# stefan01/Fusion-Method-for-Video-Frame-Interpolation

Measured on AMD Instinct MI355X. Metric: interpolated frames/sec at 1080p, higher is better.
Workload: dtype f32; 1 GPU; full fused frame (PhaseNet + 4x AdaCoF + uncertainty maps + FusionNet, output_baseline) at 1920x1080, BASELINE.json configs[3]; one frame pair per rank per step; weights=random-init, 22940546 params broadcast from rank 0, frames_in_flight_per_gpu=3, hip_graph=False

## Files before the change

### fusion-method-for-video-frame-interpolation_amd/csrc/vfi_adacof.hip

```cpp
#include "vfi_grad_common.h"

#include <cstdlib>

namespace {

using vfi::ceil_div;

template <int VEC>
struct Vec;
template <>
struct Vec<1> {
    float v[1];
    __device__ __forceinline__ void load(const float *p) { v[0] = *p; }
};
template <>
struct Vec<4> {
    float v[4];
    __device__ __forceinline__ void load(const float *p) {
        const float4 t = *reinterpret_cast<const float4 *>(p);
        v[0] = t.x; v[1] = t.y; v[2] = t.z; v[3] = t.w;
    }
};

template <>
// ... 100 lines not shown
    float acc[VEC][C];
#pragma unroll
    for (int v = 0; v < VEC; ++v)
#pragma unroll
        for (int c = 0; c < C; ++c) acc[v][c] = 0.0f;

    for (int k = 0; k < F; ++k)
        for (int l = 0; l < F; ++l) {
            const size_t t = tbase + (size_t)(k * F + l) * plane;
            Vec<VEC> w, a, b;
            w.load(weight + t);
            a.load(offset_i + t);
            b.load(offset_j + t);
#pragma unroll
            for (int v = 0; v < VEC; ++v)
                tap_accumulate<C>(in, in_plane, Hin, Win, y + k * dil, x0 + v + l * dil, w.v[v],
                                  a.v[v], b.v[v], acc[v]);
        }
#pragma unroll
    for (int c = 0; c < C; ++c) {
        if (c0 + c < Ctot) {
            float o[VEC];
#pragma unroll
            for (int v = 0; v < VEC; ++v) o[v] = acc[v][c];
            store_vec<VEC>(output + ((size_t)n * Ctot + c0 + c) * plane + pix, o);
        }
    }
}

struct FlowStats {
    float m, q;
};

template <int C, int VEC, int FT, int UNROLL_L, int MIN_WAVES, bool RGBX = false, bool SOFTMAX = false, bool WIN = false>
__global__ __launch_bounds__(256, MIN_WAVES) void adacof_fused_kernel(
    const float *__restrict__ frame0, const float *__restrict__ frame2,
    const float *__restrict__ w1, const float *__restrict__ a1, const float *__restrict__ b1,
    const float *__restrict__ w2, const float *__restrict__ a2, const float *__restrict__ b2,
    const float *__restrict__ occ, float *__restrict__ out_t1, float *__restrict__ out_t2,
    float *__restrict__ out_frame, float *__restrict__ out_mask, int H, int W, int Frt, int dil, int margin) {
    const int F = FT > 0 ? FT : Frt;
    const int x0 = (blockIdx.x * 64 + threadIdx.x) * VEC;
    const int y = blockIdx.y * 4 + threadIdx.y;
    const int n = blockIdx.z;
    extern __shared__ float4 win_lds[];
    const int WH = 4 + (F - 1) * dil + 2 * margin + 1, WW = 64 + (F - 1) * dil + 2 * margin + 1;
    const int yb = blockIdx.y * 4 - ((F - 1) * dil) / 2 - margin, xb = blockIdx.x * 64 - ((F - 1) * dil) / 2 - margin;
    if constexpr (WIN) {
        const int tid = threadIdx.y * 64 + threadIdx.x;
        const float4 *g0 = reinterpret_cast<const float4 *>(frame0) + (size_t)n * H * W;
        const float4 *g2 = reinterpret_cast<const float4 *>(frame2) + (size_t)n * H * W;
        for (int e = tid; e < WH * WW; e += 256) {
            const int gy = min(max(yb + e / WW, 0), H - 1), gx = min(max(xb + e % WW, 0), W - 1);
            win_lds[e] = g0[gy * W + gx];
            win_lds[WH * WW + e] = g2[gy * W + gx];
        }
        __syncthreads();
    }
    if (x0 >= W || y >= H) return;
    const size_t plane = (size_t)H * W;
    const size_t pix = (size_t)y * W + x0;
    const size_t tbase = (size_t)n * F * F * plane + pix;
    const int pad = ((F - 1) * dil) / 2;

    float res[2][VEC][C];
    float var[2][VEC];
    float acc[VEC][C], s[VEC], pa[VEC], pb[VEC], mx[VEC];
    FlowStats sa[VEC], sb[VEC];
    auto side_begin = [&](const Vec<VEC> &a0, const Vec<VEC> &b0) {
#pragma unroll
        for (int v = 0; v < VEC; ++v) {
#pragma unroll
            for (int c = 0; c < C; ++c) acc[v][c] = 0.0f;
// ... 112 lines not shown
#pragma unroll
            for (int l = 0; l < FT; ++l) { cw[l] = nw[l]; ca[l] = na[l]; cb[l] = nb[l]; }
        }
    } else {
#pragma unroll
        for (int side = 0; side < 2; ++side) {
            const float *__restrict__ in = (side ? frame2 : frame0) + (size_t)n * (RGBX ? 4 : C) * plane;
            const float *__restrict__ wp = side ? w2 : w1;
            const float *__restrict__ ap = side ? a2 : a1;
            const float *__restrict__ bp = side ? b2 : b1;
            {
                Vec<VEC> a, b;
                a.load(ap + tbase);
                b.load(bp + tbase);
                side_begin(a, b);
            }
#pragma unroll 1
            for (int k = 0; k < F; ++k)
#pragma unroll UNROLL_L
                for (int l = 0; l < F; ++l) {
                    const size_t t = tbase + (size_t)(k * F + l) * plane;
                    Vec<VEC> w, a, b;
                    w.load(wp + t);
                    a.load(ap + t);
                    b.load(bp + t);
                    tap(side, in, k, l, w, a, b);
                }
            side_end(res[side], var[side]);
        }
    }

    Vec<VEC> o;
    o.load(occ + (size_t)n * plane + pix);
#pragma unroll
    for (int c = 0; c < C; ++c) {
        const size_t q = ((size_t)n * C + c) * plane + pix;
        float f[VEC], t1[VEC], t2[VEC];
#pragma unroll
        for (int v = 0; v < VEC; ++v) {
            t1[v] = res[0][v][c];
            t2[v] = res[1][v][c];
            f[v] = o.v[v] * t1[v] + (1.0f - o.v[v]) * t2[v];
        }
        store_vec<VEC>(out_frame + q, f);
        if (out_t1) store_vec<VEC>(out_t1 + q, t1);
        if (out_t2) store_vec<VEC>(out_t2 + q, t2);
    }
    if (out_mask) {
        float m[VEC];
#pragma unroll
        for (int v = 0; v < VEC; ++v) {
            const float mx = fmaxf(var[0][v], var[1][v]);
            m[v] = fminf(fmaxf(mx, 0.0f), 20.0f) / 20.0f;
        }
        store_vec<VEC>(out_mask + (size_t)n * plane + pix, m);
    }
}

template <int CT>
__device__ __forceinline__ void tap_gradient(const float *__restrict__ in, size_t in_plane, int C, int Hin, int Win,
                                             int row, int col, float alpha, float beta, const float *dreg,
                                             const float *__restrict__ dglob, size_t plane, float &gw, float &sa,
                                             float &sb) {
    const int A = (int)alpha;
    const int B = (int)beta;
    const float fa = alpha - (float)A;
// ... 104 lines not shown
                                   float *grad_offset_i, float *grad_offset_j, int N, int C, int Hin, int Win,
                                   int H, int W, int F, int dilation, vfi_stream_t stream) {
    const bool want_off = grad_offset_i || grad_offset_j;
    VFI_REQUIRE(grad_weight || want_off, VFI_ERR_INVALID_ARG, "vfi_adacof_backward: no gradient requested");
    VFI_REQUIRE(grad_output && input && offset_i && offset_j && (weight || !want_off), VFI_ERR_INVALID_ARG,
                "vfi_adacof_backward: null pointer");
    VFI_REQUIRE(N > 0 && C > 0 && H > 0 && W > 0 && F > 0 && dilation > 0, VFI_ERR_INVALID_ARG,
                "vfi_adacof_backward: non-positive size");
    VFI_REQUIRE(Hin - ((F - 1) * dilation + 1) == H - 1 && Win - ((F - 1) * dilation + 1) == W - 1,
                VFI_ERR_SHAPE, "vfi_adacof_backward: input %dx%d does not match output %dx%d for F=%d dilation=%d",
                Hin, Win, H, W, F, dilation);
    VFI_REQUIRE((long long)Hin * Win < (1ll << 31) && (long long)N * F * F * H * W < (1ll << 40) &&
                    (long long)N * C * Hin * Win < (1ll << 40),
                VFI_ERR_UNSUPPORTED, "vfi_adacof_backward: tensor too large");
    if (!want_off) weight = nullptr;
    hipStream_t s = vfi::as_stream(stream);
    dim3 block(64, 4);
    dim3 grid(vfi::ceil_div(W, 64), vfi::ceil_div(H, 4), N);
    VFI_REQUIRE(grid.z <= 65535 && grid.y <= 65535, VFI_ERR_UNSUPPORTED, "vfi_adacof_backward: grid too large");
#define LAUNCH(CT)                                                                                           \
    hipLaunchKernelGGL((adacof_backward_kernel<CT, 1>), grid, block, 0, s, grad_output, input, weight, offset_i, \
                       offset_j, grad_weight, grad_offset_i, grad_offset_j, C, Hin, Win, H, W, F, dilation)
    if (C == 3) LAUNCH(3);
    else if (C == 1) LAUNCH(1);
    else LAUNCH(0);
#undef LAUNCH
    return vfi::check_launch("vfi_adacof_backward");
}

static int adacof_fused_impl(const float *frame0, const float *frame2, const float *w1,
                             const float *a1, const float *b1, const float *w2, const float *a2,
                             const float *b2, const float *occ, float *out_t1, float *out_t2,
                             float *out_frame, float *out_mask, int N, int C, int H, int W, int F,
                             int dilation, bool rgbx, bool softmax, vfi_stream_t stream) {
    VFI_REQUIRE(frame0 && frame2 && w1 && a1 && b1 && w2 && a2 && b2 && occ && out_frame,
                VFI_ERR_INVALID_ARG, "vfi_adacof_fused: null pointer");
    VFI_REQUIRE(N > 0 && H > 0 && W > 0 && F > 0 && dilation > 0, VFI_ERR_INVALID_ARG,
                "vfi_adacof_fused: non-positive size");
    VFI_REQUIRE(C == 3, VFI_ERR_UNSUPPORTED, "vfi_adacof_fused: C=%d (only 3 colour channels)", C);
    VFI_REQUIRE(((F - 1) * dilation) % 2 == 0, VFI_ERR_SHAPE,
                "vfi_adacof_fused: (F-1)*dilation must be even (F=%d dilation=%d)", F, dilation);
    VFI_REQUIRE((long long)H * W < (1ll << 31), VFI_ERR_UNSUPPORTED, "vfi_adacof_fused: frame too large");
    bool al16 = aligned16(occ) && aligned16(out_frame);
    for (const void *p : {(const void *)w1, (const void *)a1, (const void *)b1, (const void *)w2,
                          (const void *)a2, (const void *)b2})
        al16 = al16 && aligned16(p);
    for (const void *p : {(const void *)out_t1, (const void *)out_t2, (const void *)out_mask})
        al16 = al16 && (p == nullptr || aligned16(p));
    static const int variant = getenv("VFI_ADACOF_VARIANT") ? atoi(getenv("VFI_ADACOF_VARIANT")) : 2;
    int vec = (al16 && W % 4 == 0) ? 4 : ((al16 && W % 2 == 0) ? 2 : 1);
    if (variant == 1 && vec == 4) vec = 2;
    if (variant == 2 || rgbx) vec = 1;
    if (rgbx) VFI_REQUIRE(aligned16(frame0) && aligned16(frame2), VFI_ERR_INVALID_ARG, "vfi_adacof_fused_rgbx: frames must be 16-B aligned");
    hipStream_t s = vfi::as_stream(stream);
    dim3 block(64, 4);
    dim3 grid(vfi::ceil_div(W, 64 * vec), vfi::ceil_div(H, 4), N);
    VFI_REQUIRE(grid.z <= 65535 && grid.y <= 65535, VFI_ERR_UNSUPPORTED, "vfi_adacof_fused: grid too large");
#define LAUNCH(VEC, FT, UN, MW)                                                                          \
    hipLaunchKernelGGL((adacof_fused_kernel<3, VEC, FT, UN, MW>), grid, block, 0, s, frame0, frame2, w1, a1, b1, \
                       w2, a2, b2, occ, out_t1, out_t2, out_frame, out_mask, H, W, F, dilation, 0)
    if (softmax) VFI_REQUIRE(rgbx, VFI_ERR_UNSUPPORTED, "vfi_adacof_fused: softmax folding needs the rgbx entry point");
    static const int win_margin = getenv("VFI_ADACOF_MARGIN") ? atoi(getenv("VFI_ADACOF_MARGIN")) : 4;
    const int wh = 4 + (F - 1) * dilation + 2 * win_margin + 1, ww = 64 + (F - 1) * dilation + 2 * win_margin + 1;
    const size_t win_bytes = 2ull * wh * ww * sizeof(float4);
    if (rgbx && win_margin > 0 && win_bytes <= 64 * 1024) {
#define LAUNCH_WIN(FT, UN, SM)                                                                                       \
    hipLaunchKernelGGL((adacof_fused_kernel<3, 1, FT, UN, 3, true, SM, true>), grid, block, win_bytes, s, frame0, frame2, w1, \
                       a1, b1, w2, a2, b2, occ, out_t1, out_t2, out_frame, out_mask, H, W, F, dilation, win_margin)
        if (F == 5) { if (softmax) LAUNCH_WIN(5, 5, true); else LAUNCH_WIN(5, 5, false); }
        else        { if (softmax) LAUNCH_WIN(0, 1, true); else LAUNCH_WIN(0, 1, false); }
#undef LAUNCH_WIN
    } else if (rgbx) {
        if (F == 5 && softmax)
            hipLaunchKernelGGL((adacof_fused_kernel<3, 1, 5, 5, 3, true, true>), grid, block, 0, s, frame0, frame2, w1, a1, b1,
                               w2, a2, b2, occ, out_t1, out_t2, out_frame, out_mask, H, W, F, dilation, 0);
        else if (softmax)
            hipLaunchKernelGGL((adacof_fused_kernel<3, 1, 0, 1, 4, true, true>), grid, block, 0, s, frame0, frame2, w1, a1, b1,
                               w2, a2, b2, occ, out_t1, out_t2, out_frame, out_mask, H, W, F, dilation, 0);
        else if (F == 5)
            hipLaunchKernelGGL((adacof_fused_kernel<3, 1, 5, 5, 3, true>), grid, block, 0, s, frame0, frame2, w1, a1, b1,
                               w2, a2, b2, occ, out_t1, out_t2, out_frame, out_mask, H, W, F, dilation, 0);
        else
            hipLaunchKernelGGL((adacof_fused_kernel<3, 1, 0, 1, 4, true>), grid, block, 0, s, frame0, frame2, w1, a1, b1,
                               w2, a2, b2, occ, out_t1, out_t2, out_frame, out_mask, H, W, F, dilation, 0);
    } else if (F == 5) {
        if (vec == 4) LAUNCH(4, 5, 1, 3);
        else if (vec == 2) LAUNCH(2, 5, 1, 4);
        else LAUNCH(1, 5, 5, 3);
    } else {
        if (vec == 4) LAUNCH(4, 0, 1, 3); else if (vec == 2) LAUNCH(2, 0, 1, 4); else LAUNCH(1, 0, 1, 4);
    }
#undef LAUNCH
    return vfi::check_launch("vfi_adacof_fused");
}

extern "C" int vfi_adacof_fused(const float *frame0, const float *frame2, const float *w1,
                                const float *a1, const float *b1, const float *w2, const float *a2,
                                const float *b2, const float *occ, float *out_t1, float *out_t2,
                                float *out_frame, float *out_mask, int N, int C, int H, int W, int F,
                                int dilation, vfi_stream_t stream) {
    return adacof_fused_impl(frame0, frame2, w1, a1, b1, w2, a2, b2, occ, out_t1, out_t2, out_frame, out_mask, N, C,
                             H, W, F, dilation, false, false, stream);
}

extern "C" int vfi_adacof_fused_rgbx(const float *frame0_rgbx, const float *frame2_rgbx, const float *w1,
                                     const float *a1, const float *b1, const float *w2, const float *a2,
                                     const float *b2, const float *occ, float *out_t1, float *out_t2,
                                     float *out_frame, float *out_mask, int N, int H, int W, int F,
                                     int dilation, int weights_are_logits, vfi_stream_t stream) {
    return adacof_fused_impl(frame0_rgbx, frame2_rgbx, w1, a1, b1, w2, a2, b2, occ, out_t1, out_t2, out_frame,
                             out_mask, N, 3, H, W, F, dilation, true, weights_are_logits != 0, stream);
}
```

### fusion-method-for-video-frame-interpolation_amd/csrc/vfi_aux.hip

```cpp
#include "vfi_grad_common.h"

namespace {

using vfi::ceil_div;

__global__ void adacof_prepare_kernel(const float *__restrict__ f0, const float *__restrict__ f2,
                                      float *__restrict__ p0, float *__restrict__ p2, float *__restrict__ x6,
                                      int N, int H, int W, int Hp, int Wp, int rgbx) {
    const long long total = (long long)N * 3 * Hp * Wp;
    for (long long i = (long long)blockIdx.x * blockDim.x + threadIdx.x; i < total; i += (long long)gridDim.x * blockDim.x) {
        const int x = i % Wp, y = (i / Wp) % Hp, c = (i / ((long long)Wp * Hp)) % 3, n = i / ((long long)Wp * Hp * 3);
        const int sy = y < H ? y : 2 * (H - 1) - y, sx = x < W ? x : 2 * (W - 1) - x;
        const size_t s = (((size_t)n * 3 + c) * H + sy) * W + sx;
        const float mean = c == 0 ? 0.4631f : (c == 1 ? 0.4352f : 0.3990f);
        const float a = f0[s], b = f2[s];
        const size_t plane = (size_t)Hp * Wp, pix = (size_t)y * Wp + x;
        if (rgbx) {
            p0[((size_t)n * plane + pix) * 4 + c] = a;
            p2[((size_t)n * plane + pix) * 4 + c] = b;
        } else {
            p0[i] = a;
            p2[i] = b;
        }
        x6[((size_t)n * 6 + c) * plane + pix] = a - mean;
        x6[((size_t)n * 6 + 3 + c) * plane + pix] = b - mean;
    }
}

template <bool MAX>
__global__ void pool2_kernel(const float *__restrict__ x, long long x_bs, float *__restrict__ y, long long y_bs,
                             int N, int C, int H, int W) {
    const int Ho = H / 2, Wo = W / 2;
    const long long total = (long long)N * C * Ho * Wo;
    for (long long i = (long long)blockIdx.x * blockDim.x + threadIdx.x; i < total; i += (long long)gridDim.x * blockDim.x) {
        const int xo = i % Wo, yo = (i / Wo) % Ho, c = (i / ((long long)Wo * Ho)) % C, n = i / ((long long)Wo * Ho * C);
        const float *p = x + (size_t)n * x_bs + ((size_t)c * H + 2 * yo) * W + 2 * xo;
        const float2 r0 = *reinterpret_cast<const float2 *>(p);
        const float2 r1 = *reinterpret_cast<const float2 *>(p + W);
        const float v = MAX ? fmaxf(fmaxf(r0.x, r0.y), fmaxf(r1.x, r1.y)) : (r0.x + r0.y + r1.x + r1.y) * 0.25f;
        y[(size_t)n * y_bs + ((size_t)c * Ho + yo) * Wo + xo] = v;
    }
}
template <bool MAX>
__global__ void pool2_kernel_unaligned(const float *__restrict__ x, long long x_bs, float *__restrict__ y,
                                       long long y_bs, int N, int C, int H, int W) {
    const int Ho = H / 2, Wo = W / 2;
    const long long total = (long long)N * C * Ho * Wo;
    for (long long i = (long long)blockIdx.x * blockDim.x + threadIdx.x; i < total; i += (long long)gridDim.x * blockDim.x) {
        const int xo = i % Wo, yo = (i / Wo) % Ho, c = (i / ((long long)Wo * Ho)) % C, n = i / ((long long)Wo * Ho * C);
        const float *p = x + (size_t)n * x_bs + ((size_t)c * H + 2 * yo) * W + 2 * xo;
        const float a = p[0], b = p[1], cc = p[W], d = p[W + 1];
        const float v = MAX ? fmaxf(fmaxf(a, b), fmaxf(cc, d)) : (a + b + cc + d) * 0.25f;
        y[(size_t)n * y_bs + ((size_t)c * Ho + yo) * Wo + xo] = v;
    }
}
// ... 262 lines not shown
}
__global__ void phasenet_emit_low_fuse_kernel(const float *__restrict__ pred, long long pred_bs, const float *__restrict__ low,
                                              long long low_bs, const float *__restrict__ maxv, float *__restrict__ out,
                                              int N, int HW) {
    const long long total = (long long)N * HW;
    for (long long i = (long long)blockIdx.x * blockDim.x + threadIdx.x; i < total; i += (long long)gridDim.x * blockDim.x) {
        const int p = i % HW, n = i / HW;
        const float *pr = pred + (size_t)n * pred_bs + p;
        const float alpha = (pr[0] + 1.0f) / 2.0f, fa = (pr[HW] + 1.0f) / 2.0f;
        const float *l = low + (size_t)n * low_bs + p;
        const float two = alpha * l[0] + (1.0f - alpha) * l[HW];
        out[i] = (fa * two + (1.0f - fa) * l[(size_t)2 * HW]) * maxv[n];
    }
}

__global__ void tanh_residual_clamp_kernel(const float *__restrict__ x, const float *__restrict__ base,
                                           float *__restrict__ y, long long total) {
    for (long long i = (long long)blockIdx.x * blockDim.x + threadIdx.x; i < total; i += (long long)gridDim.x * blockDim.x)
        y[i] = fminf(fmaxf(base[i] + tanhf(x[i]), 0.0f), 1.0f);
}

}

extern "C" int vfi_adacof_prepare(const float *frame0, const float *frame2, float *pad0, float *pad2, float *x6,
                                  int N, int H, int W, int Hp, int Wp, int rgbx, vfi_stream_t stream) {
    VFI_REQUIRE(frame0 && frame2 && pad0 && pad2 && x6, VFI_ERR_INVALID_ARG, "vfi_adacof_prepare: null pointer");
    VFI_REQUIRE(N > 0 && H > 0 && W > 0 && Hp >= H && Wp >= W, VFI_ERR_INVALID_ARG, "vfi_adacof_prepare: bad sizes");
    VFI_REQUIRE(Hp - H < H && Wp - W < W, VFI_ERR_SHAPE, "vfi_adacof_prepare: reflect pad %dx%d needs a larger frame than %dx%d",
                Hp - H, Wp - W, H, W);
    LAUNCH_1D(adacof_prepare_kernel, (long long)N * 3 * Hp * Wp, stream, frame0, frame2, pad0, pad2, x6, N, H, W, Hp, Wp, rgbx);
    return vfi::check_launch("vfi_adacof_prepare");
}

extern "C" int vfi_pool2(const float *x, long long x_bstride, float *y, long long y_bstride, int N, int C, int H,
                         int W, int is_max, vfi_stream_t stream) {
    VFI_REQUIRE(x && y, VFI_ERR_INVALID_ARG, "vfi_pool2: null pointer");
    VFI_REQUIRE(N > 0 && C > 0 && H >= 2 && W >= 2, VFI_ERR_INVALID_ARG, "vfi_pool2: bad sizes");
    const long long total = (long long)N * C * (H / 2) * (W / 2);
    const bool al = (W % 2 == 0) && ((reinterpret_cast<uintptr_t>(x) & 7u) == 0) && (x_bstride % 2 == 0);
    if (al) {
        if (is_max) LAUNCH_1D(pool2_kernel<true>, total, stream, x, x_bstride, y, y_bstride, N, C, H, W);
        else LAUNCH_1D(pool2_kernel<false>, total, stream, x, x_bstride, y, y_bstride, N, C, H, W);
    } else {
        if (is_max) LAUNCH_1D(pool2_kernel_unaligned<true>, total, stream, x, x_bstride, y, y_bstride, N, C, H, W);
        else LAUNCH_1D(pool2_kernel_unaligned<false>, total, stream, x, x_bstride, y, y_bstride, N, C, H, W);
    }
    return vfi::check_launch("vfi_pool2");
}

extern "C" int vfi_resize_bilinear(const float *x, long long x_bstride, const float *residual, long long res_bstride,
                                   float *y, long long y_bstride, int N, int C, int Hin, int Win, int Hout, int Wout,
                                   int align_corners, int relu_input, vfi_stream_t stream) {
    VFI_REQUIRE(x && y, VFI_ERR_INVALID_ARG, "vfi_resize_bilinear: null pointer");
    VFI_REQUIRE(N > 0 && C > 0 && Hin > 0 && Win > 0 && Hout > 0 && Wout > 0, VFI_ERR_INVALID_ARG,
                "vfi_resize_bilinear: bad sizes");
    const bool vec = Wout % 4 == 0 && (reinterpret_cast<uintptr_t>(y) & 15u) == 0 && y_bstride % 4 == 0 &&
                     (!residual || ((reinterpret_cast<uintptr_t>(residual) & 15u) == 0 && res_bstride % 4 == 0));
    VFI_REQUIRE((long long)N * C <= 65535, VFI_ERR_UNSUPPORTED, "vfi_resize_bilinear: N*C = %lld planes", (long long)N * C);
    const dim3 block(64, 4), grid(ceil_div(vec ? Wout / 4 : Wout, 64), ceil_div(Hout, 4), N * C);
    if (Hin <= Hout && Win <= Wout && Hout >= kRsTileY && Wout >= 64) {
        const dim3 tgrid(ceil_div(Wout, kRsTileX), ceil_div(Hout, kRsTileY), N * C);
        if (vec)
            hipLaunchKernelGGL(resize_bilinear_tile_kernel<true>, tgrid, dim3(256), 0, vfi::as_stream(stream), x, x_bstride, residual,
                               res_bstride, y, y_bstride, C, Hin, Win, Hout, Wout, align_corners, relu_input);
        else
            hipLaunchKernelGGL(resize_bilinear_tile_kernel<false>, tgrid, dim3(256), 0, vfi::as_stream(stream), x, x_bstride, residual,
// ... 108 lines not shown
```

### fusion-method-for-video-frame-interpolation_amd/csrc/vfi_conv.hip

```cpp
#include "vfi_conv_common.h"

#include <cstdlib>

using namespace vfi::conv;

namespace {

using f32x16 = __attribute__((ext_vector_type(16))) float;


__device__ float g_zero_word = 0.0f;



template <int KS, int CK, int NT, int RW = 2>
struct ConvTile {
    static constexpr int TH = 4 * RW, TW = 32, PADK = (KS - 1) / 2;
    static constexpr int R = TH + KS - 1, PW = TW + KS - 1, PLANE = R * PW, TAPS = KS * KS, BN = 32 * NT;
    static constexpr int IN_ELEMS = CK * PLANE;
    static constexpr int IN_ELEMS_PAD = (IN_ELEMS + 3) / 4 * 4;
    static constexpr int W_ELEMS = CK * TAPS * BN;
    static constexpr int IN_PER_THREAD = (IN_ELEMS + 255) / 256;
    static constexpr int W4_PER_THREAD = (W_ELEMS / 4 + 255) / 256;
    static constexpr int W_ALLOC = (W_ELEMS + 255) / 256 * 256;
// ... 350 lines not shown
    vec *yp = reinterpret_cast<vec *>(y + (size_t)blockIdx.y * y_bs) + q;
#pragma unroll
    for (int o = 0; o < NOUT; ++o) {
        if (o < Cout) {
            const float b = bias ? bias[o] : 0.0f;
            vec r;
#pragma unroll
            for (int k = 0; k < VEC; ++k) r[k] = apply_act(acc[o][k] + b, a_);
            yp[(size_t)o * plane] = r;
        }
    }
}

static int conv1x1_stream_vec(const ConvArgs &a, int KS) {
    static const bool on = !(getenv("VFI_CONV_STREAM1X1") && atoi(getenv("VFI_CONV_STREAM1X1")) == 0);
    const long long HW = (long long)a.H * a.W;
    if (!on || KS != 1 || a.Cout > 16 || a.res || HW < 4096) return 0;
    const uintptr_t bits = reinterpret_cast<uintptr_t>(a.x) | reinterpret_cast<uintptr_t>(a.y) | (uintptr_t)(a.x_bs * 4) | (uintptr_t)(a.y_bs * 4) |
                           (uintptr_t)(HW * 4);
    return (bits & 15u) == 0 ? 4 : (bits & 7u) == 0 ? 2 : 0;
}

template <int NOUT, int VEC>
static int launch_conv1x1_stream(const ConvArgs &a, int N, hipStream_t s) {
    const int HW = a.H * a.W;
    const dim3 grid((unsigned)vfi::ceil_div(HW / VEC, 256), (unsigned)N);
    if (a.act == 3)
        hipLaunchKernelGGL((conv1x1_stream_kernel<3, NOUT, VEC>), grid, dim3(256), 0, s, a.x, a.x_bs, a.wp, a.bias, a.y, a.y_bs, a.Cin, a.Cout, a.Cout_pad, HW, a.act);
    else
        hipLaunchKernelGGL((conv1x1_stream_kernel<-1, NOUT, VEC>), grid, dim3(256), 0, s, a.x, a.x_bs, a.wp, a.bias, a.y, a.y_bs, a.Cin, a.Cout, a.Cout_pad, HW, a.act);
    return vfi::check_launch("vfi_conv2d");
}

template <int VEC>
__global__ __launch_bounds__(256) void phasenet_predict_kernel(const float *__restrict__ x, long long x_bs, const float *__restrict__ wp,
                                                               const float *__restrict__ bias, int Cout_pad, const float *__restrict__ amp_in,
                                                               long long amp_bs, const float *__restrict__ maxv, float *__restrict__ pred,
                                                               long long pred_bs, float *__restrict__ phase_out, float *__restrict__ amp_out,
                                                               int Cin, int HW) {
    typedef float vec __attribute__((ext_vector_type(VEC)));
    const int q = blockIdx.x * 256 + threadIdx.x;
    if (q * VEC >= HW) return;
    const int n = blockIdx.y;
    const vec *xp = reinterpret_cast<const vec *>(x + (size_t)n * x_bs) + q;
    const size_t plane = (size_t)HW / VEC;
    float acc[8][VEC];
#pragma unroll
    for (int o = 0; o < 8; ++o)
#pragma unroll
        for (int k = 0; k < VEC; ++k) acc[o][k] = 0.0f;
    int c = 0;
    for (; c + 8 <= Cin; c += 8) {
        vec v[8];
#pragma unroll
        for (int i = 0; i < 8; ++i) v[i] = xp[(size_t)(c + i) * plane];
#pragma unroll
        for (int i = 0; i < 8; ++i) {
            const float *w = wp + (size_t)(c + i) * Cout_pad;
#pragma unroll
            for (int o = 0; o < 8; ++o) {
                const float wo = w[o];
#pragma unroll
                for (int k = 0; k < VEC; ++k) acc[o][k] = fmaf(wo, v[i][k], acc[o][k]);
            }
        }
    }
    for (; c < Cin; ++c) {
        const vec v = xp[(size_t)c * plane];
        const float *w = wp + (size_t)c * Cout_pad;
#pragma unroll
        for (int o = 0; o < 8; ++o) {
            const float wo = w[o];
#pragma unroll
            for (int k = 0; k < VEC; ++k) acc[o][k] = fmaf(wo, v[k], acc[o][k]);
        }
    }
    vec *pp = reinterpret_cast<vec *>(pred + (size_t)n * pred_bs) + q;
#pragma unroll
    for (int o = 0; o < 8; ++o) {
        const float b = bias ? bias[o] : 0.0f;
        vec r;
#pragma unroll
        for (int k = 0; k < VEC; ++k) r[k] = acc[o][k] = apply_act(acc[o][k] + b, 3);
        pp[(size_t)o * plane] = r;
    }
    const vec *ap = reinterpret_cast<const vec *>(amp_in + (size_t)n * amp_bs) + q;
    vec *pho = reinterpret_cast<vec *>(phase_out + (size_t)n * 4 * HW) + q, *amo = reinterpret_cast<vec *>(amp_out + (size_t)n * 4 * HW) + q;
    const float mx = maxv[n];
#pragma unroll
    for (int b = 0; b < 4; ++b) {
        const vec a0 = ap[(size_t)b * plane], a1 = ap[(size_t)(4 + b) * plane];
        vec ph, am;
#pragma unroll
        for (int k = 0; k < VEC; ++k) {
            const float beta = (acc[4 + b][k] + 1.0f) / 2.0f;
            const float a = fmaf(beta, a1[k], (1.0f - beta) * a0[k]);
            ph[k] = acc[b][k] * 3.14159265358979323846f;
            am[k] = a * mx;
        }
        pho[(size_t)b * plane] = ph;
        amo[(size_t)b * plane] = am;
    }
}

template <int VEC>
__global__ __launch_bounds__(256) void phasenet_predict_fuse_kernel(const float *__restrict__ x, long long x_bs, const float *__restrict__ wp,
                                                                    const float *__restrict__ bias, int Cout_pad, const float *__restrict__ amp_in,
                                                                    long long amp_bs, const float *__restrict__ maxv, float *__restrict__ pred,
                                                                    long long pred_bs, float *__restrict__ phase_out, float *__restrict__ amp_out,
                                                                    int Cin, int HW) {
    typedef float vec __attribute__((ext_vector_type(VEC)));
    constexpr int NOUT = 12;
    const int q = blockIdx.x * 256 + threadIdx.x;
    if (q * VEC >= HW) return;
    const int n = blockIdx.y;
    const vec *xp = reinterpret_cast<const vec *>(x + (size_t)n * x_bs) + q;
    const size_t plane = (size_t)HW / VEC;
// ... 70 lines not shown
        hipLaunchKernelGGL(conv2d_splitk_reduce_kernel<1>, dim3(vfi::ceil_div(HW, 256), b.Cout, N), dim3(256), 0, s, b.ws,
                           b.splits, b.bias, b.res, b.res_bs, b.y, b.y_bs, b.Cout, HW, b.act);
}

extern "C" long long vfi_conv2d_packed_floats(int Cout, int Cin, int KS) {
    if (Cout <= 0 || Cin <= 0 || KS <= 0) return -1;
    return (long long)round_up(Cin, 8) * (KS * KS + (KS == 3 ? 16 + 36 : 0)) * round_up(Cout, 32);
}

extern "C" int vfi_conv2d_pack(const float *w_oihw, const float *scale, float *packed, int Cout, int Cin,
                               int KS, vfi_stream_t stream) {
    VFI_REQUIRE(w_oihw && packed, VFI_ERR_INVALID_ARG, "vfi_conv2d_pack: null pointer");
    VFI_REQUIRE(Cout > 0 && Cin > 0 && (KS == 1 || KS == 3 || KS == 5), VFI_ERR_INVALID_ARG,
                "vfi_conv2d_pack: bad shape Cout=%d Cin=%d KS=%d", Cout, Cin, KS);
    const int Cin_pad = round_up(Cin, 8), Cout_pad = round_up(Cout, 32);
    const long long total = (long long)Cin_pad * KS * KS * Cout_pad;
    const int blocks = (int)((total + 255) / 256 < 4096 ? (total + 255) / 256 : 4096);
    hipLaunchKernelGGL(conv2d_pack_kernel, dim3(blocks), dim3(256), 0, vfi::as_stream(stream), w_oihw, scale,
                       packed, Cout, Cin, KS * KS, Cin_pad, Cout_pad);
    if (KS == 3) {
        launch_pack_winograd(w_oihw, scale, packed + total, Cout, Cin, Cin_pad, Cout_pad, vfi::as_stream(stream));
        launch_pack_winograd4(w_oihw, scale, packed + total + (long long)Cin_pad * 16 * Cout_pad, Cout, Cin, Cin_pad, Cout_pad,
                              vfi::as_stream(stream));
    }
    return vfi::check_launch("vfi_conv2d_pack");
}

static int conv2d_impl(const float *x, long long x_bstride, const float *packed_w, const float *bias,
                       const float *residual, long long res_bstride, float *y, long long y_bstride, int N,
                       int Cin, int H, int W, int Cout, int KS, int pad_mode, int act, bool ups, float *workspace,
                       long long workspace_floats, vfi_stream_t stream, const float *x2 = nullptr, long long x2_bstride = 0,
                       int rsz_channels = 0, int Hs = 0, int Ws = 0, float *pooled = nullptr, long long pooled_bstride = 0,
                       int pool_max = 0) {
    VFI_REQUIRE(x && packed_w && y, VFI_ERR_INVALID_ARG, "vfi_conv2d: null pointer");
    VFI_REQUIRE(N > 0 && Cin > 0 && Cout > 0 && H > 0 && W > 0, VFI_ERR_INVALID_ARG, "vfi_conv2d: non-positive size");
    VFI_REQUIRE(KS == 1 || KS == 3 || KS == 5, VFI_ERR_UNSUPPORTED, "vfi_conv2d: kernel size %d", KS);
    VFI_REQUIRE(pad_mode == 0 || pad_mode == 1, VFI_ERR_INVALID_ARG, "vfi_conv2d: pad_mode %d", pad_mode);
    VFI_REQUIRE(act >= 0 && act <= 4, VFI_ERR_INVALID_ARG, "vfi_conv2d: act %d", act);
    VFI_REQUIRE(pad_mode == 0 || ((KS - 1) / 2 < H && (KS - 1) / 2 < W), VFI_ERR_SHAPE,
                "vfi_conv2d: reflect padding %d needs a larger input than %dx%d", (KS - 1) / 2, H, W);
    VFI_REQUIRE((long long)Cin * H * W < (1ll << 31) && (long long)Cout * H * W < (1ll << 31), VFI_ERR_UNSUPPORTED,
                "vfi_conv2d: per-sample tensor too large for 32-bit offsets");
    VFI_REQUIRE(N <= 65535, VFI_ERR_UNSUPPORTED, "vfi_conv2d: batch %d", N);
    ConvArgs a;
    a.x = x; a.wp = packed_w; a.bias = bias; a.res = residual; a.y = y;
    a.x_bs = x_bstride; a.res_bs = res_bstride; a.y_bs = y_bstride;
    a.Cin = Cin; a.Cin_pad = round_up(Cin, 8); a.Cout = Cout; a.Cout_pad = round_up(Cout, 32);
    a.H = H; a.W = W; a.tiles_x = vfi::ceil_div(W, 32);
    a.pad_mode = pad_mode; a.act = act;
    a.ws = workspace_floats > 0 ? workspace : nullptr; a.ws_floats = workspace ? workspace_floats : 0; a.splits = 1;
    a.x2 = nullptr; a.x2_bs = 0; a.rsz_channels = 0; a.wino_tiles = 0; a.wino_items = 0; a.wino_batch = 0; a.wino_run = 1;
    a.Hs = H / 2; a.Ws = W / 2;
    a.pool = nullptr; a.pool_bs = 0; a.pool_max = pool_max;
    a.ups_sy = H > 1 ? (float)(a.Hs - 1) / (float)(H - 1) : 0.0f;
    a.ups_sx = W > 1 ? (float)(a.Ws - 1) / (float)(W - 1) : 0.0f;
    hipStream_t s = vfi::as_stream(stream);
    const bool wide = (a.Cout_pad % 64 == 0);
    if (ups) {
        VFI_REQUIRE(KS == 3 && pad_mode == 0 && H % 2 == 0 && W % 2 == 0 && H < 65536 && W < 65536, VFI_ERR_UNSUPPORTED,
                    "vfi_conv2d_upsample2x: needs KS=3, zero padding, even output size (got KS=%d pad=%d %dx%d)", KS, pad_mode, H, W);
        return wide ? launch_conv<3, 8, 2, 1>(a, N, s) : launch_conv<3, 8, 1, 1>(a, N, s);
    }
    if (x2) {
        VFI_REQUIRE(KS == 3 && wide && rsz_channels > 0 && rsz_channels % 8 == 0 && rsz_channels <= Cin && Hs > 0 && Ws > 0 &&
                    H < 65536 && W < 65536, VFI_ERR_UNSUPPORTED,
                    "vfi_conv2d_resized_prefix: needs KS=3, Cout%%64==0, prefix channels a multiple of 8 (got KS=%d Cout=%d prefix=%d)",
                    KS, Cout, rsz_channels);
        a.x2 = x2; a.x2_bs = x2_bstride; a.rsz_channels = rsz_channels; a.Hs = Hs; a.Ws = Ws;
        a.ups_sy = (float)Hs / (float)H; a.ups_sx = (float)Ws / (float)W;
        return launch_conv<3, 8, 2, 2>(a, N, s);
    }
    static const bool wino_on = !(getenv("VFI_CONV_WINOGRAD") && atoi(getenv("VFI_CONV_WINOGRAD")) == 0);
    const long long wino_work_items = (long long)a.tiles_x * vfi::ceil_div(H, 8) * N * (a.Cout_pad / 32) * 16;
    if (KS == 3 && wino_on && (long long)Cin * H * W * 4 < (1ll << 32) && wino_work_items < (1ll << 30)) {
        a.pool = pooled; a.pool_bs = pooled_bstride;
        if (winograd4_suits(a, N)) {
            a.wp = packed_w + (size_t)a.Cin_pad * (9 + 16) * a.Cout_pad;
            return launch_winograd4(a, N, s);
        }
        a.wp = packed_w + (size_t)a.Cin_pad * 9 * a.Cout_pad;
        return launch_winograd(a, N, s);
    }
    if (pooled) {
        const int rc = conv2d_impl(x, x_bstride, packed_w, bias, residual, res_bstride, y, y_bstride, N, Cin, H, W, Cout, KS, pad_mode,
                                   act, false, workspace, workspace_floats, stream);
        return rc ? rc : vfi_pool2(y, y_bstride, pooled, pooled_bstride, N, Cout, H, W, pool_max, stream);
    }
    if (const int vec = conv1x1_stream_vec(a, KS)) {
        if (a.Cout <= 8) return vec == 4 ? launch_conv1x1_stream<8, 4>(a, N, s) : launch_conv1x1_stream<8, 2>(a, N, s);
        return vec == 4 ? launch_conv1x1_stream<16, 4>(a, N, s) : launch_conv1x1_stream<16, 2>(a, N, s);
    }
    if (KS == 3) return wide ? launch_conv<3, 8, 2>(a, N, s) : launch_conv<3, 8, 1>(a, N, s);
    if (KS == 5) return wide ? launch_conv<5, 4, 2>(a, N, s) : launch_conv<5, 4, 1>(a, N, s);
    return wide ? launch_conv<1, 8, 2>(a, N, s) : launch_conv<1, 8, 1>(a, N, s);
}

extern "C" int vfi_conv2d_algo(int N, int Cin, int H, int W, int Cout, int KS, int has_residual, int pooled, int act) {
    if (N < 1 || Cin < 1 || H < 1 || W < 1 || Cout < 1) return VFI_ERR_INVALID_ARG;
    if (KS != 1 && KS != 3 && KS != 5) return VFI_ERR_UNSUPPORTED;
    if (KS == 1) {
        ConvArgs q{};
        q.Cout = Cout; q.H = H; q.W = W;
        static float dummy1;
        q.res = has_residual ? &dummy1 : nullptr;
        return conv1x1_stream_vec(q, KS) ? VFI_CONV_ALGO_STREAM1X1 : VFI_CONV_ALGO_DIRECT;
    }
    static const bool wino_on = !(getenv("VFI_CONV_WINOGRAD") && atoi(getenv("VFI_CONV_WINOGRAD")) == 0);
    ConvArgs a{};
    a.Cin = Cin; a.Cout = Cout; a.Cout_pad = round_up(Cout, 32); a.H = H; a.W = W; a.act = act; a.tiles_x = vfi::ceil_div(W, 32);
    static float dummy;
    a.res = has_residual ? &dummy : nullptr;
    a.pool = pooled ? &dummy : nullptr;
    const long long wino_work_items = (long long)a.tiles_x * vfi::ceil_div(H, 8) * N * (a.Cout_pad / 32) * 16;
    if (KS == 3 && wino_on && (long long)Cin * H * W * 4 < (1ll << 32) && wino_work_items < (1ll << 30))
        return winograd4_suits(a, N) ? VFI_CONV_ALGO_WINOGRAD4 : VFI_CONV_ALGO_WINOGRAD2;
    return VFI_CONV_ALGO_DIRECT;
}

extern "C" int vfi_conv2d(const float *x, long long x_bstride, const float *packed_w, const float *bias,
                          const float *residual, long long res_bstride, float *y, long long y_bstride, int N,
                          int Cin, int H, int W, int Cout, int KS, int pad_mode, int act, float *workspace,
                          long long workspace_floats, vfi_stream_t stream) {
    return conv2d_impl(x, x_bstride, packed_w, bias, residual, res_bstride, y, y_bstride, N, Cin, H, W, Cout, KS,
                       pad_mode, act, false, workspace, workspace_floats, stream);
}

extern "C" int vfi_phasenet_predict(const float *feat, long long feat_bstride, const float *packed_w, const float *bias,
                                    const float *amp_in, long long amp_bstride, const float *max_amp, float *pred, long long pred_bstride,
                                    float *phase_out, float *amp_out, int N, int Cin, int H, int W, vfi_stream_t stream) {
    VFI_REQUIRE(feat && packed_w && amp_in && max_amp && pred && phase_out && amp_out, VFI_ERR_INVALID_ARG, "vfi_phasenet_predict: null pointer");
    VFI_REQUIRE(N > 0 && N <= 65535 && Cin > 0 && H > 0 && W > 0, VFI_ERR_INVALID_ARG, "vfi_phasenet_predict: bad sizes");
    const long long HW = (long long)H * W;
    VFI_REQUIRE((long long)Cin * HW < (1ll << 31), VFI_ERR_UNSUPPORTED, "vfi_phasenet_predict: per-sample tensor too large for 32-bit offsets");
    ConvArgs a{};
    a.x = feat; a.y = pred; a.x_bs = feat_bstride; a.y_bs = pred_bstride; a.Cout = 8; a.H = H; a.W = W;
    int vec = conv1x1_stream_vec(a, 1);
    const uintptr_t bits = reinterpret_cast<uintptr_t>(amp_in) | reinterpret_cast<uintptr_t>(phase_out) | reinterpret_cast<uintptr_t>(amp_out) | (uintptr_t)(amp_bstride * 4);
    if (vec == 4 && (bits & 15u)) vec = (bits & 7u) ? 0 : 2;
    else if (vec == 2 && (bits & 7u)) vec = 0;
    if (!vec) {
        const int rc = conv2d_impl(feat, feat_bstride, packed_w, bias, nullptr, 0, pred, pred_bstride, N, Cin, H, W, 8, 1, 0, 3, false, nullptr, 0, stream);
        return rc ? rc : vfi_phasenet_emit(pred, pred_bstride, amp_in, amp_bstride, max_amp, phase_out, amp_out, N, (int)HW, stream);
    }
    const dim3 grid((unsigned)vfi::ceil_div((int)(HW / vec), 256), (unsigned)N);
    hipStream_t s = vfi::as_stream(stream);
    if (vec == 4)
        hipLaunchKernelGGL(phasenet_predict_kernel<4>, grid, dim3(256), 0, s, feat, feat_bstride, packed_w, bias, 32, amp_in, amp_bstride, max_amp, pred,
                           pred_bstride, phase_out, amp_out, Cin, (int)HW);
    else
        hipLaunchKernelGGL(phasenet_predict_kernel<2>, grid, dim3(256), 0, s, feat, feat_bstride, packed_w, bias, 32, amp_in, amp_bstride, max_amp, pred,
                           pred_bstride, phase_out, amp_out, Cin, (int)HW);
    return vfi::check_launch("vfi_phasenet_predict");
}

extern "C" int vfi_phasenet_predict_n(const float *feat, long long feat_bstride, const float *packed_w, const float *bias,
                                      const float *amp_in, long long amp_bstride, const float *max_amp, float *pred, long long pred_bstride,
                                      float *phase_out, float *amp_out, int N, int Cin, int H, int W, int num_img, vfi_stream_t stream) {
    VFI_REQUIRE(feat && packed_w && amp_in && max_amp && pred && phase_out && amp_out, VFI_ERR_INVALID_ARG, "vfi_phasenet_predict_n: null pointer");
    VFI_REQUIRE(N > 0 && N <= 65535 && Cin > 0 && H > 0 && W > 0, VFI_ERR_INVALID_ARG, "vfi_phasenet_predict_n: bad sizes");
    VFI_REQUIRE(num_img >= 2 && num_img <= 4, VFI_ERR_UNSUPPORTED, "vfi_phasenet_predict_n: num_img %d (2, 3 or 4)", num_img);
    if (num_img != 3)
        return vfi_phasenet_predict(feat, feat_bstride, packed_w, bias, amp_in, amp_bstride, max_amp, pred, pred_bstride, phase_out, amp_out, N,
                                    Cin, H, W, stream);
    const long long HW = (long long)H * W;
    VFI_REQUIRE((long long)Cin * HW < (1ll << 31), VFI_ERR_UNSUPPORTED, "vfi_phasenet_predict_n: per-sample tensor too large for 32-bit offsets");
    ConvArgs a{};
    a.x = feat; a.y = pred; a.x_bs = feat_bstride; a.y_bs = pred_bstride; a.Cout = 12; a.H = H; a.W = W;
    int vec = conv1x1_stream_vec(a, 1);
    const uintptr_t bits = reinterpret_cast<uintptr_t>(amp_in) | reinterpret_cast<uintptr_t>(phase_out) | reinterpret_cast<uintptr_t>(amp_out) | (uintptr_t)(amp_bstride * 4);
    if (vec == 4 && (bits & 15u)) vec = (bits & 7u) ? 0 : 2;
    else if (vec == 2 && (bits & 7u)) vec = 0;
    if (!vec) {
        const int rc = conv2d_impl(feat, feat_bstride, packed_w, bias, nullptr, 0, pred, pred_bstride, N, Cin, H, W, 12, 1, 0, 3, false, nullptr, 0, stream);
        return rc ? rc : vfi_phasenet_emit_n(pred, pred_bstride, amp_in, amp_bstride, max_amp, phase_out, amp_out, N, (int)HW, 3, stream);
    }
    const dim3 grid((unsigned)vfi::ceil_div((int)(HW / vec), 256), (unsigned)N);
    hipStream_t s = vfi::as_stream(stream);
    if (vec == 4)
        hipLaunchKernelGGL(phasenet_predict_fuse_kernel<4>, grid, dim3(256), 0, s, feat, feat_bstride, packed_w, bias, 32, amp_in, amp_bstride, max_amp, pred,
// ... 35 lines not shown
```

### fusion-method-for-video-frame-interpolation_amd/csrc/vfi_conv_winograd.hip

```cpp
#include "vfi_conv_common.h"

using namespace vfi::conv;

namespace {

using f32x4 = __attribute__((ext_vector_type(4))) float;

struct WinoTile {
    static constexpr int TH = 8, TW = 32, R = TH + 2, CK = 4, BN = 32;
    static constexpr int ROWP = 36;
    static constexpr int PLANE = R * ROWP;
    static constexpr int PLANE_S = (PLANE - 32 + 63) / 64 * 64 + 32;
    static constexpr int PIECES = PLANE_S / 4;
    static constexpr int IN_X4 = (CK * PIECES + 255) / 256;
    static constexpr int IN_X1 = (CK * PLANE_S + 255) / 256;
    static constexpr int IN_FLOATS = IN_X4 * 1024;
    static constexpr int W_FLOATS = CK * 16 * BN, W_INSTR = W_FLOATS / 4 / 256;
    static constexpr int BUF = IN_FLOATS + W_FLOATS;
    static constexpr int NBUF = 4;
    static constexpr int MIN_LOADS = IN_X4 + W_INSTR;
    static constexpr int BIAS_SLOTS = 8;
    static constexpr int BIAS_OFF = NBUF * BUF;
    static constexpr size_t LDS_BYTES = ((size_t)NBUF * BUF + BIAS_SLOTS * 64) * sizeof(float);
    static_assert(IN_X1 * 256 <= IN_FLOATS && PLANE_S % 4 == 0 && ROWP % 4 == 0 && BIAS_SLOTS > NBUF, "tile layout");
// ... 195 lines not shown
    }
    zero_acc();
    while (true) {
        fetch_u(u23, slot, 2);
        __builtin_amdgcn_sched_barrier(0);
        mfma_rows(u01, v, 0);
        __builtin_amdgcn_sched_barrier(0);
        asm volatile("s_waitcnt vmcnt(8) lgkmcnt(0)" ::: "memory");
        __builtin_amdgcn_s_barrier();
        asm volatile("" ::: "memory");
        __builtin_amdgcn_sched_barrier(0);
        const int cur_slot = slot;
        slot = slot + 1 == T::NBUF ? 0 : slot + 1;
        float d[4][4];
        fetch_d(d, slot);
        fetch_u(u01, slot, 0);
        __builtin_amdgcn_sched_barrier(0);
        mfma_rows(u23, v, 2);
        __builtin_amdgcn_sched_barrier(0);
        __builtin_amdgcn_s_setprio(3);
        issue_next(cur_slot);
        transform(d, v);
        __builtin_amdgcn_s_setprio(0);
        const bool last_of_item = ch + 1 == ch_end;
        const int nL = last_of_item ? next_valid(cL + G) : cL;
        const bool more = nL < Ltotal;
        ++ch;
        if (last_of_item) {
            const int gxw = it.x0 + 2 * n16, gy0 = it.y0 + 2 * wave;
            const bool split_out = a.splits > 1;
            const float *__restrict__ resp = (RES && !split_out && a.res) ? a.res + (size_t)it.n * a.res_bs : nullptr;
            float *__restrict__ yp = split_out ? a.ws + ((size_t)it.split * N + it.n) * a.Cout * HW : a.y + (size_t)it.n * a.y_bs;
            const int act = ACT >= 0 ? ACT : (split_out ? 0 : a.act);
            const int co0 = it.nb * T::BN + 4 * k4;
            const float *bias_l = lds + T::BIAS_OFF + (cseq & (T::BIAS_SLOTS - 1)) * 64 + 4 * k4;
            auto outputs = [&](int mb, int j, float2 (&o)[2]) {
                float s0[4], s1[4];
#pragma unroll
                for (int c = 0; c < 4; ++c) {
                    s0[c] = acc[mb][c][j] + acc[mb][4 + c][j] + acc[mb][8 + c][j];
                    s1[c] = acc[mb][4 + c][j] - acc[mb][8 + c][j] - acc[mb][12 + c][j];
                }
                o[0] = make_float2(s0[0] + s0[1] + s0[2], s0[1] - s0[2] - s0[3]);
                o[1] = make_float2(s1[0] + s1[1] + s1[2], s1[1] - s1[2] - s1[3]);
            };
            const bool vec4 = it.x0 + T::TW <= a.W && it.y0 + T::TH <= a.H && (a.W % 4 == 0) && ((reinterpret_cast<size_t>(yp) & 15) == 0) &&
                              (!resp || (reinterpret_cast<size_t>(resp) & 15) == 0);
            const int Hq = a.H >> 1, Wq = a.W >> 1;
            float *__restrict__ pq = POOL ? a.pool + (size_t)it.n * a.pool_bs + (size_t)co0 * Hq * Wq + (size_t)(gy0 >> 1) * Wq + (gxw >> 1) : nullptr;
            const bool pool_ok = POOL && (gy0 >> 1) < Hq && (gxw >> 1) < Wq;
            auto pooled = [&](const float2 (&o)[2], float b) {
                const float p0 = apply_act(o[0].x + b, act), p1 = apply_act(o[0].y + b, act);
                const float p2 = apply_act(o[1].x + b, act), p3 = apply_act(o[1].y + b, act);
                return a.pool_max ? fmaxf(fmaxf(p0, p1), fmaxf(p2, p3)) : (p0 + p1 + p2 + p3) * 0.25f;
            };
            if (vec4) {
                const bool odd = n16 & 1;
                const size_t off = (size_t)co0 * HW + (size_t)(gy0 + (odd ? 1 : 0)) * a.W + (gxw & ~3);
#pragma unroll
                for (int mb = 0; mb < 2; ++mb)
#pragma unroll
                    for (int j = 0; j < 4; ++j) {
                        const int dc = mb * 16 + j;
                        float2 o[2];
                        outputs(mb, j, o);
                        if (POOL && pool_ok && co0 + dc < a.Cout) pq[(size_t)dc * Hq * Wq] = pooled(o, bias_l[dc]);
                        const float2 give = odd ? o[0] : o[1];
                        float2 got;
                        got.x = __builtin_bit_cast(float, __builtin_amdgcn_update_dpp(0, __builtin_bit_cast(int, give.x), 0xB1, 0xf, 0xf, false));
                        got.y = __builtin_bit_cast(float, __builtin_amdgcn_update_dpp(0, __builtin_bit_cast(int, give.y), 0xB1, 0xf, 0xf, false));
                        float4 q = odd ? make_float4(got.x, got.y, o[1].x, o[1].y) : make_float4(o[0].x, o[0].y, got.x, got.y);
                        const float b = split_out ? 0.0f : bias_l[dc];
                        q.x = apply_act(q.x + b, act); q.y = apply_act(q.y + b, act);
                        q.z = apply_act(q.z + b, act); q.w = apply_act(q.w + b, act);
                        if (co0 + dc < a.Cout) {
                            if (RES && resp) {
                                const float4 r = *reinterpret_cast<const float4 *>(resp + off + (size_t)dc * HW);
                                q.x += r.x; q.y += r.y; q.z += r.z; q.w += r.w;
                            }
                            *reinterpret_cast<float4 *>(yp + off + (size_t)dc * HW) = q;
                        }
                    }
            } else if (gy0 < a.H && gxw < a.W) {
                const size_t off = (size_t)co0 * HW + (size_t)gy0 * a.W + gxw;
#pragma unroll
                for (int mb = 0; mb < 2; ++mb)
#pragma unroll
                    for (int j = 0; j < 4; ++j) {
                        const int dc = mb * 16 + j;
                        if (co0 + dc >= a.Cout) continue;
                        float2 o[2];
                        outputs(mb, j, o);
                        const float b = split_out ? 0.0f : bias_l[dc];
                        if (POOL && pool_ok) pq[(size_t)dc * Hq * Wq] = pooled(o, b);
#pragma unroll
                        for (int dy = 0; dy < 2; ++dy)
                            if (gy0 + dy < a.H) {
                                const size_t e = off + (size_t)dc * HW + (size_t)dy * a.W;
                                float vx = apply_act(o[dy].x + b, act), vy = apply_act(o[dy].y + b, act);
                                if (RES && resp) {
                                    vx += resp[e];
                                    if (gxw + 1 < a.W) vy += resp[e + 1];
                                }
                                yp[e] = vx;
                                if (gxw + 1 < a.W) yp[e + 1] = vy;
                            }
                    }
            }
            if (!more) break;
            cL = nL;
            ++cseq;
            it = decode_item(a, cL);
            ch = fast_div(nchunks_all * it.split, a.fd_splits);
            ch_end = fast_div(nchunks_all * (it.split + 1), a.fd_splits);
            zero_acc();
        }
    }
    asm volatile("s_waitcnt vmcnt(0)" ::: "memory");
}

__global__ void conv2d_pack_winograd_kernel(const float *__restrict__ w, const float *__restrict__ scale,
                                            float *__restrict__ out, int Cout, int Cin, int Cin_pad, int Cout_pad) {
    const size_t total = (size_t)Cin_pad * 16 * Cout_pad;
    for (size_t e = (size_t)blockIdx.x * blockDim.x + threadIdx.x; e < total; e += (size_t)gridDim.x * blockDim.x) {
        const int j = e & 3, co = (e >> 2) % Cout_pad, i = (e / ((size_t)4 * Cout_pad)) & 3, ci = e / ((size_t)16 * Cout_pad);
        double u = 0.0;
        if (co < Cout && ci < Cin) {
            const float *g = w + ((size_t)co * Cin + ci) * 9;
            const double G[4][3] = {{1.0, 0.0, 0.0}, {0.5, 0.5, 0.5}, {0.5, -0.5, 0.5}, {0.0, 0.0, 1.0}};
            for (int r = 0; r < 3; ++r)
// ... 34 lines not shown
        resident = 2 * cus;
    }
    ConvArgs b = a;
    const int cb = a.Cout_pad / T::BN;
    b.wino_tiles = a.tiles_x * vfi::ceil_div(a.H, T::TH);
    b.wino_batch = N;
    b.wino_run = 1;
    while (b.wino_run < 8 && (long long)b.wino_tiles * N >= 256ll * 2 * b.wino_run) b.wino_run *= 2;
    b.wino_items = round_up(b.wino_tiles * N, 8 * b.wino_run) * cb;
    b.splits = 1;
    const int nchunks = vfi::ceil_div(a.Cin, T::CK);
    const long long out_floats = (long long)N * a.Cout * a.H * a.W;
    if (a.ws && nchunks >= 16 && b.wino_items < 4 * resident) {
        auto cost = [&](int S) {
            const double rounds = (double)(((long long)b.wino_items * S + resident - 1) / resident);
            const double reduce = S > 1 ? 4.0 + (double)(S + 1) * out_floats * 4.0 / 2.5e6 : 0.0;
            return rounds * (1.1 * nchunks / S) + reduce;
        };
        int best = 1;
        for (int S = 2; S <= 16; S *= 2)
            if (nchunks / S >= 8 && out_floats * S <= a.ws_floats && cost(S) < cost(best)) best = S;
        if (cost(best) <= 0.9 * cost(1)) b.splits = best;
    }
    b.fd_items = make_fastdiv((unsigned)b.wino_items);
    b.fd_cb = make_fastdiv((unsigned)cb);
    b.fd_run = make_fastdiv((unsigned)b.wino_run);
    b.fd_tiles = make_fastdiv((unsigned)b.wino_tiles);
    b.fd_tiles_x = make_fastdiv((unsigned)b.tiles_x);
    b.fd_splits = make_fastdiv((unsigned)b.splits);
    const long long items = (long long)b.wino_items * b.splits;
    dim3 grid(capped_grid(items < resident ? items : resident));
    const int act = b.splits > 1 ? 0 : b.act;
    const bool pool_fused = b.pool && b.splits == 1 && !b.res && act == 1;
    if (pool_fused) {
        hipLaunchKernelGGL((conv3x3_winograd_kernel<false, 1, true>), grid, dim3(256), T::LDS_BYTES, s, b);
        return vfi::check_launch("vfi_conv2d");
    }
    if (b.res && b.splits == 1) hipLaunchKernelGGL((conv3x3_winograd_kernel<true, -1>), grid, dim3(256), T::LDS_BYTES, s, b);
    else if (act == 0) hipLaunchKernelGGL((conv3x3_winograd_kernel<false, 0>), grid, dim3(256), T::LDS_BYTES, s, b);
    else if (act == 1) hipLaunchKernelGGL((conv3x3_winograd_kernel<false, 1>), grid, dim3(256), T::LDS_BYTES, s, b);
    else if (act == 2) hipLaunchKernelGGL((conv3x3_winograd_kernel<false, 2>), grid, dim3(256), T::LDS_BYTES, s, b);
    else if (act == 3) hipLaunchKernelGGL((conv3x3_winograd_kernel<false, 3>), grid, dim3(256), T::LDS_BYTES, s, b);
    else hipLaunchKernelGGL((conv3x3_winograd_kernel<false, 4>), grid, dim3(256), T::LDS_BYTES, s, b);
    if (b.splits > 1) launch_splitk_reduce(b, N, s);
    if (b.pool) {
        const int rc = vfi_pool2(b.y, b.y_bs, b.pool, b.pool_bs, N, b.Cout, b.H, b.W, b.pool_max, s);
        if (rc) return rc;
    }
    return vfi::check_launch("vfi_conv2d");
}
```

### fusion-method-for-video-frame-interpolation_amd/csrc/vfi_conv_winograd4.hip

```cpp
#include "vfi_conv_winograd4_common.h"

#include <cstdlib>

using namespace vfi::conv;

namespace {

using namespace vfi::conv::w4;

template <int ACT, bool RES = false, bool POOL = false>
__global__ __launch_bounds__(512, 2) void conv3x3_winograd4_kernel(const ConvArgs a) {
    using T = Wino4Tile;
    extern __shared__ __attribute__((aligned(16))) float lds[];
    const int tid = threadIdx.x, lane = tid & 63, wave = uni((int)(threadIdx.x >> 6));
    const int n16 = lane & 15, k4 = lane >> 4;
    const int trow = wave & 3, chalf = wave >> 2;
    const int HW = a.H * a.W, G = gridDim.x;
    const int Ltotal = a.wino_items;
    const int nchunks = (a.Cin + T::CK - 1) / T::CK;

    auto next_valid = [&](int L) __attribute__((always_inline)) {
        while (L < Ltotal && !decode_item(a, L).valid) L += G;
        return L;
    };
// ... 199 lines not shown
                for (int c = 0; c < 6; ++c) {
                    const float col[6] = {acc[c][j], acc[6 + c][j], acc[12 + c][j], acc[18 + c][j], acc[24 + c][j], acc[30 + c][j]};
                    float o[4];
                    output_transform6(col, o);
#pragma unroll
                    for (int r = 0; r < 4; ++r) tt[r][c] = o[r];
                }
                const float b = bias_l[j];
                if (co0 + j < a.Cout) {
                    const size_t plane = (size_t)(co0 + j) * HW;
                    float *pc = yp + plane;
                    float prev[4];
#pragma unroll
                    for (int r = 0; r < 4; ++r) {
                        float o[4];
                        output_transform6(tt[r], o);
#pragma unroll
                        for (int c = 0; c < 4; ++c) o[c] = apply_act(o[c] + b, act);
                        const int gy = gy0 + r;
                        if (POOL) {
                            if (r & 1) {
                                const int qy = (gy0 >> 1) + (r >> 1);
#pragma unroll
                                for (int cc = 0; cc < 2; ++cc) {
                                    const float p0 = prev[2 * cc], p1 = prev[2 * cc + 1], p2 = o[2 * cc], p3 = o[2 * cc + 1];
                                    const float pv = a.pool_max ? fmaxf(fmaxf(p0, p1), fmaxf(p2, p3)) : (p0 + p1 + p2 + p3) * 0.25f;
                                    if (qy < Hq && (gx >> 1) + cc < Wq) pq[(size_t)(co0 + j) * Hq * Wq + (size_t)(r >> 1) * Wq + cc] = pv;
                                }
                            } else {
#pragma unroll
                                for (int c = 0; c < 4; ++c) prev[c] = o[c];
                            }
                        }
                        if (gy < a.H) {
                            if (vec4) {
                                if (gx < a.W) {
                                    float4 q = make_float4(o[0], o[1], o[2], o[3]);
                                    if (RES) {
                                        const float4 rr = *reinterpret_cast<const float4 *>(resp + plane + (size_t)gy * a.W + gx);
                                        q.x += rr.x; q.y += rr.y; q.z += rr.z; q.w += rr.w;
                                    }
                                    *reinterpret_cast<float4 *>(pc + (size_t)gy * a.W + gx) = q;
                                }
                            } else {
#pragma unroll
                                for (int c = 0; c < 4; ++c)
                                    if (gx + c < a.W) pc[(size_t)gy * a.W + gx + c] = o[c] + (RES ? resp[plane + (size_t)gy * a.W + gx + c] : 0.0f);
                            }
                        }
                    }
                }
            }
            const int nL = next_valid(cL + G);
            if (nL >= Ltotal) break;
            cL = nL;
            ++cseq;
            it = decode_item(a, cL);
            ch = 0;
            zero_acc();
        }
    }
    asm volatile("s_waitcnt vmcnt(0)" ::: "memory");
}

__global__ void conv2d_pack_winograd4_kernel(const float *__restrict__ w, const float *__restrict__ scale,
                                             float *__restrict__ out, int Cout, int Cin, int Cin_pad, int Cout_pad) {
    const size_t total = (size_t)Cin_pad * 36 * Cout_pad;
// ... 102 lines not shown
```

### fusion-method-for-video-frame-interpolation_amd/csrc/vfi_conv_winograd4m.hip

```cpp
#include "vfi_conv_winograd4_common.h"
#include "vfi_conv_winograd4m_body.h"

#include <cstdlib>
#include <type_traits>
#include <utility>

using namespace vfi::conv;

namespace {

using namespace vfi::conv::w4;
#ifndef W4M_PK_EPILOGUE
#define W4M_PK_EPILOGUE 1
#endif
using f32x2 = __attribute__((ext_vector_type(2))) float;
using i32x4 = __attribute__((ext_vector_type(4))) int;
using u32x4 = __attribute__((ext_vector_type(4))) unsigned;
using u32x2 = __attribute__((ext_vector_type(2))) unsigned;

struct W4M {
    using T = Wino4Tile;
    static constexpr int THREADS = 256, WAVES = 4;
    static constexpr int IN_PIECES = T::IN_WI / WAVES;
    static constexpr int W_PIECES = (T::W_WI + WAVES - 1) / WAVES;
// ... 35 lines not shown
    d.x = __builtin_amdgcn_readfirstlane((int)(unsigned)v);
    d.y = __builtin_amdgcn_readfirstlane((int)(unsigned)(v >> 32));
    d.z = __builtin_amdgcn_readfirstlane((int)bytes);
    d.w = 0x00020000;
    return d;
}

template <int K, int E>
__device__ __forceinline__ float acc_read() {
    float x;
    if constexpr (K < 64) asm volatile("v_accvgpr_read_b32 %0, a%c1" : "=v"(x) : "i"(4 * K + E));
    else asm volatile("v_mov_b32 %0, v%c1" : "=v"(x) : "i"(W4M_ACCV + 4 * (K - 64) + E));
    return x;
}
template <int N, class F, int... I>
__device__ __forceinline__ void static_for_impl(F &&f, std::integer_sequence<int, I...>) {
    (f(std::integral_constant<int, I>{}), ...);
}
template <int N, class F>
__device__ __forceinline__ void static_for(F &&f) {
    static_for_impl<N>(static_cast<F &&>(f), std::make_integer_sequence<int, N>{});
}

#ifdef W4M_STAMPS
__device__ unsigned long long w4m_stamps[256 * 4 * 10];
extern "C" int vfi_debug_w4m_stamps(unsigned long long *host, int n) {
    return hipMemcpyFromSymbol(host, HIP_SYMBOL(w4m_stamps), sizeof(unsigned long long) * (size_t)n) == hipSuccess ? 0 : -1;
}
#define W4M_STAMP(var) var = __builtin_amdgcn_s_memtime()
#else
#define W4M_STAMP(var)
#endif

template <int ACT, bool RES = false, bool POOL = false>
__global__ __launch_bounds__(256, 1) void conv3x3_winograd4m_kernel(const ConvArgs a) {
    using T = Wino4Tile;
    extern __shared__ __attribute__((aligned(16))) float lds[];
    const int tid = threadIdx.x, lane = tid & 63, wave = uni((int)(threadIdx.x >> 6));
    const int n16 = lane & 15, k4 = lane >> 4;
    const int HW = a.H * a.W, G = gridDim.x;
    const int Ltotal = a.wino_items;
    const int nchunks = (a.Cin + T::CK - 1) / T::CK;
    const unsigned lds_base = (unsigned)(unsigned long long)(__attribute__((address_space(3))) char *)lds;

    auto next_valid = [&](int L, Item &d) __attribute__((always_inline)) {
        d = decode_item(a, L < Ltotal ? L : 0);
        while (L < Ltotal && !d.valid) {
            L += G;
            d = decode_item(a, L < Ltotal ? L : 0);
        }
        return L;
    };

#ifdef W4M_STAMPS
    unsigned long long t_epi1 = 0, t_epi2 = 0;
#endif
    State st;
    W4M_STATEMENT(ZERO, st);
    st.pa0 = lds_base + (unsigned)(k4 * T::PLANE_S + 4 * wave * T::ROWP + 4 * n16) * 4u;
    st.wa0 = lds_base + (unsigned)(T::IN_FLOATS + (k4 * T::NGRP * T::BN + n16) * 4) * 4u;
    st.s_wave = (unsigned)wave;
    st.s_five = 5.0f;
#pragma unroll
    for (int t = 0; t < 5; ++t) st.s_w[t] = (unsigned)uni((wave + W4M::WAVES * t) * 32 * a.Cout_pad);
    st.s_wstep = (unsigned)uni(W4M::WAVES * 32 * a.Cout_pad);
    st.s_wt = 0;
    st.wvoff = 0;
// ... 125 lines not shown
                rL = iL;
                rit = iit;
            } else {
                rL = next_valid(rL + G, rit);
            }
            rleft = nchunks;
            setup_read();
        }
    };

    setup_issue();
#pragma unroll
    for (int p = 0; p < W4M::AHEAD; ++p) issue_now();

    Item it;
    int cL = next_valid(blockIdx.x, it);
    if (cL >= Ltotal) {
        asm volatile("s_waitcnt vmcnt(0)" ::: "memory");
        return;
    }
    int ch = 0, cseq = 0;
    setup_read();
    W4M_STATEMENT(PRIME, st);
    advance_read();

    auto epilogue_form = [&](auto fast_tag) __attribute__((always_inline)) {
        constexpr bool FAST = decltype(fast_tag)::value;
        int ln = lane;
        asm volatile("" : "+v"(ln));
        const int n16 = ln & 15, k4 = ln >> 4;
        const int gx = it.x0 + 4 * n16, gy0 = it.y0 + 4 * wave;
        const int act = ACT >= 0 ? ACT : a.act;
        const unsigned plane_bytes = (unsigned)HW * 4u, row_bytes = (unsigned)a.W * 4u;
        const __amdgpu_buffer_rsrc_t ydesc = make_rsrc(a.y + (size_t)it.n * a.y_bs, (unsigned)a.Cout * plane_bytes);
        const __amdgpu_buffer_rsrc_t rdesc = make_rsrc(RES ? a.res + (size_t)it.n * a.res_bs : a.y, RES ? (unsigned)a.Cout * plane_bytes : 0u);
        const int Hq = a.H >> 1, Wq = a.W >> 1;
        const __amdgpu_buffer_rsrc_t pdesc = make_rsrc(POOL ? a.pool + (size_t)it.n * a.pool_bs : a.y, POOL ? (unsigned)a.Cout * (unsigned)(Hq * Wq) * 4u : 0u);
        const unsigned cbase = (unsigned)(it.nb * T::BN + 4 * k4);
        const unsigned lane_off = (cbase * (unsigned)HW + (unsigned)(gy0 * a.W + gx)) * 4u;
        const unsigned pool_off = (cbase * (unsigned)(Hq * Wq) + (unsigned)((gy0 >> 1) * Wq + (gx >> 1))) * 4u;
        const bool row4 = FAST || uni((int)((a.W & 3) == 0 || it.x0 + T::TW <= a.W)) != 0;
        const unsigned baddr = lds_base + (unsigned)(W4M::BIAS_OFF + (cseq & (W4M::BIAS_SLOTS - 1)) * 64 + 4 * k4) * 4u;
        f32x4 bias4 = {0.0f, 0.0f, 0.0f, 0.0f};
        u32x4 rres[2][4];
        if constexpr (FAST && RES) {
            const unsigned rvoff = gx < a.W ? lane_off : 0xffffffffu;
#pragma unroll
            for (int r = 0; r < 4; ++r) rres[0][r] = __builtin_amdgcn_raw_buffer_load_b128(rdesc, rvoff, (int)(r * row_bytes), 0);
        }
        static_for<8>([&](auto hj) __attribute__((always_inline)) {
            constexpr int h = decltype(hj)::value / 4, j = decltype(hj)::value % 4;
            __builtin_amdgcn_sched_barrier(0);
#ifdef W4M_STAMPS
            unsigned long long e_a, e_b, e_c;
            W4M_STAMP(e_a);
#endif
            if constexpr (j == 0) asm volatile("ds_read_b128 %0, %1 offset:%c2\n\ts_waitcnt lgkmcnt(0)" : "=&v"(bias4) : "v"(baddr), "i"(64 * h));
            if constexpr (FAST && RES) {
                constexpr int g1 = decltype(hj)::value + 1;
                if constexpr (g1 < 8) {
                    const unsigned rvoff = gx < a.W ? lane_off + (unsigned)(16 * (g1 / 4) + g1 % 4) * plane_bytes : 0xffffffffu;
#pragma unroll
                    for (int r = 0; r < 4; ++r) rres[g1 & 1][r] = __builtin_amdgcn_raw_buffer_load_b128(rdesc, rvoff, (int)(r * row_bytes), 0);
                    __builtin_amdgcn_sched_barrier(0);
                }
            }
            float tt[4][6];
// ... 31 lines not shown
            t_epi1 += e_b - e_a;
#endif
            const float b = bias4[j];
            const unsigned ch_off = (unsigned)(16 * h + j) * plane_bytes;
            const unsigned voff = gx < a.W ? lane_off + ch_off : 0xffffffffu;
            float prev[4];
#pragma unroll
            for (int r = 0; r < 4; ++r) {
                float o[4];
                output_transform6(tt[r], o);
#pragma unroll
                for (int c = 0; c < 4; ++c) o[c] = apply_act(o[c] + b, act);
                if (POOL) {
                    if (r & 1) {
                        const float q0 = a.pool_max ? fmaxf(fmaxf(prev[0], prev[1]), fmaxf(o[0], o[1])) : (prev[0] + prev[1] + o[0] + o[1]) * 0.25f;
                        const float q1 = a.pool_max ? fmaxf(fmaxf(prev[2], prev[3]), fmaxf(o[2], o[3])) : (prev[2] + prev[3] + o[2] + o[3]) * 0.25f;
                        const unsigned pch = (unsigned)(16 * h + j) * (unsigned)(Hq * Wq) * 4u + (unsigned)((r >> 1) * Wq) * 4u;
                        if (FAST) {
                            __builtin_amdgcn_raw_buffer_store_b64(u32x2{__float_as_uint(q0), __float_as_uint(q1)}, pdesc, (gx >> 1) + 1 < Wq ? pool_off + pch : 0xffffffffu, 0, 0);
                        } else if ((gy0 >> 1) + (r >> 1) < Hq) {
                            const int qx = gx >> 1;
                            if (row4) {
                                __builtin_amdgcn_raw_buffer_store_b64(u32x2{__float_as_uint(q0), __float_as_uint(q1)}, pdesc, qx + 1 < Wq ? pool_off + pch : 0xffffffffu, 0, 0);
                            } else {
                                __builtin_amdgcn_raw_buffer_store_b32(__float_as_uint(q0), pdesc, qx < Wq ? pool_off + pch : 0xffffffffu, 0, 0);
                                __builtin_amdgcn_raw_buffer_store_b32(__float_as_uint(q1), pdesc, qx + 1 < Wq ? pool_off + pch + 4u : 0xffffffffu, 0, 0);
                            }
                        }
                    } else {
#pragma unroll
                        for (int c = 0; c < 4; ++c) prev[c] = o[c];
                    }
                }
                if (FAST || gy0 + r < a.H) {
                    const int soff = (int)(r * row_bytes);
                    if (row4) {
                        if (RES) {
                            u32x4 rr;
                            if constexpr (FAST) rr = rres[(4 * h + j) & 1][r];
                            else rr = __builtin_amdgcn_raw_buffer_load_b128(rdesc, voff, soff, 0);
#pragma unroll
                            for (int c = 0; c < 4; ++c) o[c] += __uint_as_float(rr[c]);
                        }
                        __builtin_amdgcn_raw_buffer_store_b128(u32x4{__float_as_uint(o[0]), __float_as_uint(o[1]), __float_as_uint(o[2]), __float_as_uint(o[3])},
                                                               ydesc, voff, soff, 0);
                    } else {
#pragma unroll
                        for (int c = 0; c < 4; ++c) {
                            const unsigned vc = gx + c < a.W ? lane_off + ch_off + 4u * c : 0xffffffffu;
                            if (RES) o[c] += __uint_as_float(__builtin_amdgcn_raw_buffer_load_b32(rdesc, vc, soff, 0));
                            __builtin_amdgcn_raw_buffer_store_b32(__float_as_uint(o[c]), ydesc, vc, soff, 0);
                        }
                    }
                }
            }
#ifdef W4M_STAMPS
            __builtin_amdgcn_sched_barrier(0);
            W4M_STAMP(e_c);
            t_epi2 += e_c - e_b;
#endif
        });
    };
    auto epilogue = [&]() __attribute__((always_inline)) {
        W4M_STATEMENT(DRAIN, st);
        const bool fast = uni((int)(it.y0 + 4 * wave + 3 < a.H && ((a.W & 3) == 0 || it.x0 + T::TW <= a.W) && (!POOL || ((a.H | a.W) & 1) == 0))) != 0;
        if (fast) epilogue_form(std::true_type{});
        else epilogue_form(std::false_type{});
// ... 71 lines not shown
        }
        if (chunk(std::integral_constant<int, 0>{})) break;
        if (chunk(std::integral_constant<int, 1>{})) break;
    }
    asm volatile("s_waitcnt vmcnt(0) lgkmcnt(0)" ::: "memory");
#ifdef W4M_STAMPS
    if (lane == 0) {
        unsigned long long t_end;
        W4M_STAMP(t_end);
        unsigned long long *d = w4m_stamps + ((size_t)blockIdx.x * 4 + wave) * 10;
        d[8] = t_loop; d[9] = n_loop;
        d[0] = t_body; d[1] = t_between; d[2] = t_epi; d[3] = n_body; d[4] = n_epi; d[5] = t_end - t_start;
        d[6] = t_epi1; d[7] = t_epi2;
    }
#endif
}

}

bool vfi::conv::winograd4m_enabled() {
    const char *e = getenv("VFI_CONV_WINOGRAD4M");
    return !e || atoi(e) != 0;
}

int vfi::conv::launch_winograd4m(const ConvArgs &b, hipStream_t s) {
    static int resident_dev[vfi::kMaxDevices] = {};
    int &resident = resident_dev[vfi::current_device()];
    if (!resident) {
        hipError_t e = hipSuccess;
        for (const void *k : {reinterpret_cast<const void *>(conv3x3_winograd4m_kernel<0>), reinterpret_cast<const void *>(conv3x3_winograd4m_kernel<1>),
                              reinterpret_cast<const void *>(conv3x3_winograd4m_kernel<2>), reinterpret_cast<const void *>(conv3x3_winograd4m_kernel<3>),
                              reinterpret_cast<const void *>(conv3x3_winograd4m_kernel<4>), reinterpret_cast<const void *>(conv3x3_winograd4m_kernel<-1, true>),
                              reinterpret_cast<const void *>(conv3x3_winograd4m_kernel<1, true>),
                              reinterpret_cast<const void *>(conv3x3_winograd4m_kernel<1, false, true>)})
            if (e == hipSuccess) e = hipFuncSetAttribute(k, hipFuncAttributeMaxDynamicSharedMemorySize, (int)W4M::LDS_BYTES);
        int dev = 0, cus = 0;
        if (e == hipSuccess) e = hipGetDevice(&dev);
        if (e == hipSuccess) e = hipDeviceGetAttribute(&cus, hipDeviceAttributeMultiprocessorCount, dev);
        if (e != hipSuccess || cus <= 0) return vfi::fail(VFI_ERR_LAUNCH, "vfi_conv2d: Winograd F(4x4) M=32 kernel setup: %s", hipGetErrorString(e));
        resident = cus;
    }
    dim3 grid(capped_grid(b.wino_items < resident ? b.wino_items : resident));
    const size_t lds = W4M::LDS_BYTES;
    if (b.pool) hipLaunchKernelGGL((conv3x3_winograd4m_kernel<1, false, true>), grid, dim3(W4M::THREADS), lds, s, b);
    else if (b.res && b.act == 1) hipLaunchKernelGGL((conv3x3_winograd4m_kernel<1, true>), grid, dim3(W4M::THREADS), lds, s, b);
    else if (b.res) hipLaunchKernelGGL((conv3x3_winograd4m_kernel<-1, true>), grid, dim3(W4M::THREADS), lds, s, b);
    else if (b.act == 0) hipLaunchKernelGGL((conv3x3_winograd4m_kernel<0>), grid, dim3(W4M::THREADS), lds, s, b);
    else if (b.act == 1) hipLaunchKernelGGL((conv3x3_winograd4m_kernel<1>), grid, dim3(W4M::THREADS), lds, s, b);
    else if (b.act == 2) hipLaunchKernelGGL((conv3x3_winograd4m_kernel<2>), grid, dim3(W4M::THREADS), lds, s, b);
    else if (b.act == 3) hipLaunchKernelGGL((conv3x3_winograd4m_kernel<3>), grid, dim3(W4M::THREADS), lds, s, b);
    else hipLaunchKernelGGL((conv3x3_winograd4m_kernel<4>), grid, dim3(W4M::THREADS), lds, s, b);
    return vfi::check_launch("vfi_conv2d");
}
```

### fusion-method-for-video-frame-interpolation_amd/vfi_amd/_lib.py

```python
import ctypes
import os
import threading

_HERE = os.path.dirname(os.path.abspath(__file__))
_LIB_NAME = "libvfi_hip.so"

c_f = ctypes.c_void_p
c_i = ctypes.c_int
c_d = ctypes.c_double
c_s = ctypes.c_void_p
c_l = ctypes.c_longlong
c_fl = ctypes.c_float


class VfiLibraryError(RuntimeError):
    """The HIP library is missing / failed, or a tensor is not usable by it."""


SIGNATURES = {
    "vfi_debug_poison_lds": [c_s],
    "vfi_debug_conv_override": [c_i, c_i],
    "vfi_adacof_forward": [c_f] * 5 + [c_i] * 8 + [c_s],
    "vfi_adacof_backward": [c_f] * 8 + [c_i] * 8 + [c_s],
    "vfi_adacof_fused": [c_f] * 13 + [c_i] * 6 + [c_s],
    "vfi_conv2d_packed_floats": [c_i] * 3,
    "vfi_conv2d_algo": [c_i] * 9,
    "vfi_conv2d_pack": [c_f] * 3 + [c_i] * 3 + [c_s],
    "vfi_conv2d": [c_f, c_l, c_f, c_f, c_f, c_l, c_f, c_l] + [c_i] * 8 + [c_f, c_l, c_s],
    "vfi_conv2d_pool2": [c_f, c_l, c_f, c_f, c_f, c_l, c_f, c_l, c_i] + [c_i] * 8 + [c_f, c_l, c_s],
    "vfi_conv2d_upsample2x": [c_f, c_l, c_f, c_f, c_f, c_l, c_f, c_l] + [c_i] * 8 + [c_f, c_l, c_s],
    "vfi_conv2d_resized_prefix": [c_f, c_l, c_f, c_l, c_i, c_i, c_i, c_f, c_f, c_f, c_l] + [c_i] * 8 + [c_f, c_l, c_s],
    "vfi_adacof_prepare": [c_f] * 5 + [c_i] * 6 + [c_s],
    "vfi_adacof_fused_rgbx": [c_f] * 13 + [c_i] * 6 + [c_s],
    "vfi_pool2": [c_f, c_l, c_f, c_l] + [c_i] * 5 + [c_s],
    "vfi_resize_bilinear": [c_f, c_l, c_f, c_l, c_f, c_l] + [c_i] * 8 + [c_s],
    "vfi_upsample2x_tapsum": [c_f, c_f, c_i, c_i, c_i, c_fl, c_i, c_s],
    "vfi_softmax_channels": [c_f, c_l, c_f, c_l] + [c_i] * 3 + [c_s],
    "vfi_affine_slice": [c_f, c_l, c_f, c_l, c_i, c_l, c_f, c_fl, c_s],
    "vfi_batch_max": [c_f, c_l, c_i, c_l, c_fl, c_f, c_f, c_s],
    "vfi_phasenet_emit": [c_f, c_l, c_f, c_l, c_f, c_f, c_f, c_i, c_i, c_s],
    "vfi_phasenet_predict": [c_f, c_l, c_f, c_f, c_f, c_l, c_f, c_f, c_l, c_f, c_f, c_i, c_i, c_i, c_i, c_s],
    "vfi_phasenet_level_tail": [c_f, c_l, c_f, c_f, c_f, c_l, c_f, c_f, c_l, c_f, c_f, c_i, c_i, c_i, c_i, c_i, c_s],
    "vfi_phasenet_emit_low": [c_f, c_l, c_f, c_l, c_f, c_f, c_i, c_i, c_s],
    "vfi_phasenet_emit_n": [c_f, c_l, c_f, c_l, c_f, c_f, c_f, c_i, c_i, c_i, c_s],
    "vfi_phasenet_predict_n": [c_f, c_l, c_f, c_f, c_f, c_l, c_f, c_f, c_l, c_f, c_f, c_i, c_i, c_i, c_i, c_i, c_s],
    "vfi_phasenet_emit_low_n": [c_f, c_l, c_f, c_l, c_f, c_f, c_i, c_i, c_i, c_s],
    "vfi_tanh_residual_clamp": [c_f, c_f, c_f, c_l, c_s],
    "vfi_rgb2lab": [c_f, c_f, c_i, c_i, c_s],
    "vfi_lab2rgb": [c_f, c_f, c_i, c_i, c_s],
    "vfi_channel_mean_diff": [c_f, c_f, c_f, c_i, c_i, c_i, c_fl, c_i, c_s],
    "vfi_absdiff": [c_f, c_f, c_f, c_l, c_fl, c_i, c_s],
    "vfi_gaussian_filter": [c_f, c_f, c_f, c_i, c_i, c_i, c_fl, c_fl, c_s],
    "vfi_median_filter": [c_f, c_f, c_i, c_i, c_i, c_i, c_s],
    "vfi_diff_sums": [c_f, c_f, c_l, c_f, c_f, c_s],
    "vfi_ssim_sum": [c_f] * 5 + [c_i] * 4 + [c_fl, c_fl, c_f, c_f, c_s],
    "vfi_mul": [c_f, c_f, c_f, c_l, c_s],
    "vfi_avg_pool": [c_f, c_f, c_i, c_i, c_i, c_i, c_s],
# ... 184 lines not shown
```

### fusion-method-for-video-frame-interpolation_amd/vfi_amd/adacof/cupy_module/adacof.py

```python
import math

import torch

from ... import _lib


class FunctionAdaCoF(torch.autograd.Function):
    @staticmethod
    def forward(ctx, input, weight, offset_i, offset_j, dilation):
        ctx.dilation = dilation
        n, c, hin, win = input.shape
        f = int(math.sqrt(weight.size(1)))
        h, w = weight.size(2), weight.size(3)
        assert hin - ((f - 1) * dilation + 1) == h - 1
        assert win - ((f - 1) * dilation + 1) == w - 1
        assert input.is_contiguous()
        assert weight.is_contiguous()
        assert offset_i.is_contiguous()
        assert offset_j.is_contiguous()
        if not input.is_cuda:
            raise NotImplementedError()
        ctx.save_for_backward(input, weight, offset_i, offset_j)
        output = torch.empty((n, c, h, w), dtype=input.dtype, device=input.device)
        _lib.call("vfi_adacof_forward", _lib.dptr(input, "input"), _lib.dptr(weight, "weight"),
                  _lib.dptr(offset_i, "offset_i"), _lib.dptr(offset_j, "offset_j"),
                  _lib.dptr(output), n, c, hin, win, h, w, f, int(dilation), _lib.stream_ptr())
        return output

    @staticmethod
    def backward(ctx, grad_output):
        input, weight, offset_i, offset_j = ctx.saved_tensors
        need = ctx.needs_input_grad
        grad_input = torch.zeros_like(input) if need[0] else None
        return (grad_input, *adacof_backward(grad_output.contiguous(), input, weight, offset_i, offset_j, ctx.dilation,
                                             need[1:4]), None)


def adacof_backward(grad_output, input, weight, offset_i, offset_j, dilation, need=(True, True, True)):
    n, c, hin, win = input.shape
    f = int(math.sqrt(weight.size(1)))
    h, w = weight.size(2), weight.size(3)
    new = lambda: torch.empty((n, f * f, h, w), dtype=input.dtype, device=input.device)
    grad_weight = new() if need[0] else None
    grad_offset_i = new() if need[1] else None
    grad_offset_j = new() if need[2] else None
    n_out = sum(g is not None for g in (grad_weight, grad_offset_i, grad_offset_j))
    if n_out:
        want_off = grad_offset_i is not None or grad_offset_j is not None
        d = _lib.dptr
        _lib.call("vfi_adacof_backward", d(grad_output, "grad_output"), d(input, "input"),
                  d(weight, "weight") if want_off else None, d(offset_i, "offset_i"), d(offset_j, "offset_j"),
                  d(grad_weight), d(grad_offset_i), d(grad_offset_j), n, c, hin, win, h, w, f, int(dilation),
                  _lib.stream_ptr(),
                  work=("byte", float(n) * h * w * (4 * c + 4 * f * f * (2 + want_off + n_out)),
                        "adacof_backward_kernel"))
    return grad_weight, grad_offset_i, grad_offset_j


def adacof_fused(frame0, frame2, w1, a1, b1, w2, a2, b2, occ, dilation,
                 want_sides=True, want_mask=True, rgbx=False, weights_are_logits=False):
    if rgbx:
        n, h, w, c = frame0.shape[0], frame0.shape[1], frame0.shape[2], 3
    else:
        n, c, h, w = frame0.shape
    f = int(math.sqrt(w1.size(1)))
    new = lambda ch: torch.empty((n, ch, h, w), dtype=torch.float32, device=frame0.device)
    t1 = new(c) if want_sides else None
    t2 = new(c) if want_sides else None
    frame = new(c)
    mask = new(1) if want_mask else None
    d = _lib.dptr
    head = ("vfi_adacof_fused_rgbx",) if rgbx else ("vfi_adacof_fused",)
    dims = (n, h, w) if rgbx else (n, c, h, w)
    if weights_are_logits and not rgbx:
        raise _lib.VfiLibraryError("weights_are_logits needs rgbx frames")
    extra = (int(bool(weights_are_logits)),) if rgbx else ()
    _lib.call(*head, d(frame0, "frame0"), d(frame2, "frame2"), d(w1), d(a1), d(b1),
              d(w2), d(a2), d(b2), d(occ), d(t1), d(t2), d(frame), d(mask),
              *dims, f, int(dilation), *extra, _lib.stream_ptr(),
              work=("byte", float(n) * h * w * (6 * f * f * 4 + 4 + 2 * 4 * c + 4 * c * (3 if want_sides else 1)
                                                 + (4 if want_mask else 0)), "adacof_fused_kernel"))
    return t1, t2, frame, mask
```

### fusion-method-for-video-frame-interpolation_amd/vfi_amd/fusion_net/fusion_adacofnet.py

```python
import sys

import torch

from .. import _lib, ops
from ..adacof.cupy_module.adacof import FunctionAdaCoF, adacof_fused
from ..nn_util import ConvParams, Indexed, PackedModule

HEADS = ("moduleWeight1", "moduleAlpha1", "moduleBeta1", "moduleWeight2", "moduleAlpha2", "moduleBeta2",
         "moduleOcclusion")


def make_model(args):
    return AdaCoFNet(args).to(torch.device("cuda:{}".format(args.gpu_id)))


def _basic(cin, cout):
    return Indexed({0: ConvParams(cin, cout, 3), 2: ConvParams(cout, cout, 3), 4: ConvParams(cout, cout, 3)})


class KernelEstimation(PackedModule):
    def __init__(self, kernel_size):
        super().__init__()
        self.kernel_size = kernel_size
        k2 = kernel_size ** 2
        self.moduleConv1 = _basic(6, 32)
        self.moduleConv2 = _basic(32, 64)
        self.moduleConv3 = _basic(64, 128)
        self.moduleConv4 = _basic(128, 256)
        self.moduleConv5 = _basic(256, 512)
        self.moduleDeconv5 = _basic(512, 512)
        self.moduleUpsample5 = Indexed({1: ConvParams(512, 512, 3)})
        self.moduleDeconv4 = _basic(512, 256)
        self.moduleUpsample4 = Indexed({1: ConvParams(256, 256, 3)})
        self.moduleDeconv3 = _basic(256, 128)
        self.moduleUpsample3 = Indexed({1: ConvParams(128, 128, 3)})
        self.moduleDeconv2 = _basic(128, 64)
        self.moduleUpsample2 = Indexed({1: ConvParams(64, 64, 3)})
        for name in HEADS[:6]:
            setattr(self, name, Indexed({0: ConvParams(64, 64, 3), 2: ConvParams(64, 64, 3),
                                         4: ConvParams(64, k2, 3), 7: ConvParams(k2, k2, 3)}))
        self.moduleOcclusion = Indexed({0: ConvParams(64, 64, 3), 2: ConvParams(64, 64, 3),
                                        4: ConvParams(64, 64, 3), 7: ConvParams(64, 1, 3)})
        self.train(False)

    def _build_packed(self):
        p = {}
        for name in ("moduleConv1", "moduleConv2", "moduleConv3", "moduleConv4", "moduleConv5", "moduleDeconv5",
                     "moduleDeconv4", "moduleDeconv3", "moduleDeconv2"):
            m = getattr(self, name)
            p[name] = [self.pack(m[i]) for i in (0, 2, 4)]
        for name in ("moduleUpsample5", "moduleUpsample4", "moduleUpsample3", "moduleUpsample2"):
            p[name] = self.pack(getattr(self, name)[1])
        w = torch.cat([getattr(self, h)[0].weight for h in HEADS], 0)
        b = torch.cat([getattr(self, h)[0].bias for h in HEADS], 0)
        p["heads0"] = ops.PackedConv(w, b)
        for h in HEADS:
            m = getattr(self, h)
            p[h] = [self.pack(m[2]), self.pack(m[4]), self.pack(m[7])]
        w7 = self.moduleOcclusion[7].weight
        p["occ_taps"] = ops.PackedConv(w7[0].permute(1, 2, 0).reshape(9, -1, 1, 1).contiguous(), None)
        p["occ_bias"] = float(self.moduleOcclusion[7].bias.item())
        return p

    def _basic(self, convs, x):
        for pc in convs:
            x = ops.conv2d(x, pc, "zeros", "relu")
        return x

    def _basic_pooled(self, convs, x):
        for pc in convs[:-1]:
            x = ops.conv2d(x, pc, "zeros", "relu")
        return ops.conv2d_pool2(x, convs[-1], False, "zeros", "relu")

    def _up(self, pc, x, skip):
        return ops.conv2d(x, pc, "zeros", "relu", residual=skip, upsample2x=True)

    def forward_x6(self, x6, softmax=True):
        if softmax and self.wants_graph():
            return _KernelEstimationFunction.apply(self, x6, *self.parameters())
        p = self.packed()
        c1, q1 = self._basic_pooled(p["moduleConv1"], x6)
        c2, q2 = self._basic_pooled(p["moduleConv2"], q1)
        c3, q3 = self._basic_pooled(p["moduleConv3"], q2)
        c4, q4 = self._basic_pooled(p["moduleConv4"], q3)
        c5, q5 = self._basic_pooled(p["moduleConv5"], q4)
        x = self._basic(p["moduleDeconv5"], q5)
        x = self._up(p["moduleUpsample5"], x, c5)
        x = self._up(p["moduleUpsample4"], self._basic(p["moduleDeconv4"], x), c4)
        x = self._up(p["moduleUpsample3"], self._basic(p["moduleDeconv3"], x), c3)
        x = self._up(p["moduleUpsample2"], self._basic(p["moduleDeconv2"], x), c2)
        n, _, h, w = x.shape
        h0 = ops.conv2d(x, p["heads0"], "zeros", "relu")
        outs = []
        for i, name in enumerate(HEADS):
            c_mid, c_up, c_out = p[name]
            t = ops.conv2d(h0[:, 64 * i:64 * (i + 1)], c_mid, "zeros", "relu")
            t = ops.conv2d(t, c_up, "zeros", "relu")
            if name.startswith("moduleWeight"):
                t = ops.conv2d(t, c_out, "zeros", None, upsample2x=True)
                if softmax:
                    t = ops.softmax_channels_(t)
            elif name == "moduleOcclusion":
                taps = ops.conv2d(t, p["occ_taps"], "zeros", None)
                t = ops.new((n, 1, 2 * h, 2 * w), t)
                _lib.call("vfi_upsample2x_tapsum", taps.data_ptr(), t.data_ptr(), n, h, w, p["occ_bias"], 4,
                          _lib.stream_ptr())
            else:
                t = ops.conv2d(t, c_out, "zeros", None, upsample2x=True)
            outs.append(t)
        return tuple(outs)

    def forward(self, rfield0, rfield2):
        return self.forward_x6(torch.cat([rfield0, rfield2], 1).contiguous())

# ... 136 lines not shown
        return w1, a1, b1, w2, a2, b2, occ

    @staticmethod
    def backward(ctx, *g):
        net = ctx.net
        w1, a1, b1, w2, a2, b2, occ = ctx.saved_tensors[-7:]
        g = [t.contiguous() for t in g]
        gl1, ga1, gb1 = ops.adacof_head_backward(g[0], g[1], g[2], w1, a1, b1)
        gl2, ga2, gb2 = ops.adacof_head_backward(g[3], g[4], g[5], w2, a2, b2)
        gz = ops.sigmoid_backward(g[6], occ)
        names = [k for k, _ in net.named_parameters()]
        need = {k: bool(f) for k, f in zip(names, ctx.needs_input_grad[2:])}
        grads = net.backward_train(ctx.keep, (gl1, ga1, gb1, gl2, ga2, gb2, gz), need)
        ctx.keep = None
        return (None, None, *[grads.get(k) if need[k] else None for k in names])


class AdaCoFNet(torch.nn.Module):
    def __init__(self, args):
        super().__init__()
        self.args = args
        self.kernel_size = args.kernel_size
        self.kernel_pad = int(((args.kernel_size - 1) * args.dilation) / 2.0)
        self.dilation = args.dilation
        self.get_kernel = KernelEstimation(self.kernel_size)
        self.moduleAdaCoF = FunctionAdaCoF.apply
        self.train(False)

    def train(self, mode=True):
        if mode:
            raise NotImplementedError("vfi_amd implements the inference path only (eval mode)")
        return super().train(False)

    def forward(self, frame0, frame2, return_sides=True):
        h0, w0 = int(frame0.shape[2]), int(frame0.shape[3])
        if h0 != int(frame2.shape[2]) or w0 != int(frame2.shape[3]):
            sys.exit("Frame sizes do not match")
        pad0, pad2, x6 = ops.adacof_prepare(frame0.contiguous(), frame2.contiguous(), rgbx=True)
        w1, a1, b1, w2, a2, b2, occ = self.get_kernel.forward_x6(x6, softmax=False)
        t1, t2, frame1, mask = adacof_fused(pad0, pad2, w1, a1, b1, w2, a2, b2, occ, self.dilation, rgbx=True,
                                            weights_are_logits=True, want_sides=bool(return_sides))
        if x6.shape[2] != h0 or x6.shape[3] != w0:
            t1, t2, frame1, mask = (t[:, :, :h0, :w0].contiguous() if t is not None else None for t in (t1, t2, frame1, mask))
        return t1, t2, frame1, mask
```

### fusion-method-for-video-frame-interpolation_amd/vfi_amd/fusion_net/fusion_net.py

```python
import torch

from .. import ops
from ..nn_util import ConvParams, Indexed, PackedModule


class FusionNet(PackedModule):
    def __init__(self, num_imgs=5, uncertainty_maps=3, kernel=3, pad=3, dil=3):
        super().__init__()
        cin = 3 * num_imgs + uncertainty_maps
        self.in_channels = cin
        self.net = Indexed({0: ConvParams(cin, 64, kernel), 2: ConvParams(64, 64, kernel),
                            4: ConvParams(64, 64, kernel), 6: ConvParams(64, 3, kernel)})
        self.encoder_layers = Indexed({0: ConvParams(cin, 32, 5), 1: ConvParams(32, 64, 5), 2: ConvParams(64, 128, 3)})
        self.bottleneck_layer = ConvParams(128, 128, 3)
        self.decoder_layers = Indexed({0: ConvParams(128, 64, 5), 1: ConvParams(64, 32, 5), 2: ConvParams(32, 3, 1)})
        self.residuals = []
        self.train(False)

    def _build_packed(self):
        return {"enc": [self.pack(self.encoder_layers[i]) for i in range(3)],
                "mid": self.pack(self.bottleneck_layer),
                "dec": [self.pack(self.decoder_layers[i]) for i in range(3)]}

    def _live_convs(self):
        return [self.encoder_layers[i] for i in range(3)] + [self.bottleneck_layer] + [self.decoder_layers[i] for i in range(3)]

    def packed_transposed(self):
        p = self.packed()
        if "T" not in p:
            with torch.no_grad():
                p["T"] = [ops.packed_transposed(c.weight) for c in self._live_convs()]
            dev = next(self.parameters()).device
            if dev.type == "cuda":
                torch.cuda.current_stream(dev).synchronize()
        return p["T"]

    def train(self, mode=True):
        return torch.nn.Module.train(self, mode)

    def forward(self, base, adacof, phase, other, maps, save=False, variant=0):
        params = [t for c in self._live_convs() for t in (c.weight, c.bias)]
        inputs = [base, adacof, phase, other, maps]
        if torch.is_grad_enabled() and (any(t is not None and t.requires_grad for t in inputs) or
                                        (self.training and any(t.requires_grad for t in params))):
            out = _FusionNetFunction.apply(self, variant, *inputs, *params)
        else:
            out = self._forward_impl(self.packed(), base, adacof, phase, other, maps, variant, None)
        if save:
            self.residuals.append(float((out - (phase if variant == 1 else base)).sum().item()))
        return out

    def _forward_impl(self, p, base, adacof, phase, other, maps, variant, keep):
        parts = [base, adacof, phase, other] + ([maps] if maps is not None else [])
        n, _, h, w = base.shape
        if h % 8 or w % 8:
            raise ops.VfiLibraryError(f"FusionNet needs H, W multiples of 8, got {h}x{w}")
        x = ops.new((n, self.in_channels, h, w), base)
        c0 = 0
        for t in parts:
            ops.affine_slice(t.contiguous(), x[:, c0:c0 + t.shape[1]])
            c0 += t.shape[1]
        assert c0 == self.in_channels
        enc_in, skip = [x], []
        for i in range(3):
            s, x = ops.conv2d_pool2(x, p["enc"][i], True, "reflect", "relu")
            skip.append(s)
            enc_in.append(x)
        x = ops.conv2d(x, p["mid"], "reflect", None)
        dec_src, dec_in = [x], []
        for i, s in enumerate(skip[::-1]):
            x = ops.resize_bilinear(x, s.shape[2:], align_corners=False, relu_input=True, residual=s)
            dec_in.append(x)
            x = ops.conv2d(x, p["dec"][i], "reflect", None)
            dec_src.append(x)
        head_base = (phase if variant == 1 else base).contiguous()
        out = ops.tanh_residual_clamp(x, head_base)
        if keep is not None:
            keep.update(enc_in=enc_in, skip=skip, dec_src=dec_src, dec_in=dec_in, head_base=head_base,
                        widths=[t.shape[1] for t in parts])
        return out


class _FusionNetFunction(torch.autograd.Function):

    @staticmethod
    def forward(ctx, net, variant, base, adacof, phase, other, maps, *params):
        keep = {}
        out = net._forward_impl(net.packed(), base, adacof, phase, other, maps, variant, keep)
        ctx.net, ctx.variant, ctx.keep = net, variant, keep
        ctx.has_maps = maps is not None
        ctx.save_for_backward(*params)
        return out

    @staticmethod
# ... 42 lines not shown
```

### fusion-method-for-video-frame-interpolation_amd/vfi_amd/fusion_net/interpolate_twoframe.py

```python
import math
import os
from types import SimpleNamespace

import numpy as np
import torch

from .. import ops
from ..adacof.models import Model
from ..phase_net.phase_net import PhaseNet
from ..train.pyramid import Pyramid
from ..train.utils import calc_pyr_height
from ..values import DecompValues
from .fusion_net import FusionNet

DEFAULT_ADACOF_MODEL = "vfi_amd.fusion_net.fusion_adacofnet"


def crop_center(img, cropx, cropy):
    y, x, _ = img.shape
    startx = x // 2 - (cropx // 2)
    starty = y // 2 - (cropy // 2)
    return img[starty:starty + cropy, startx:startx + cropx]


def imwrite(tensor, path, range=(0, 1)):
    from PIL import Image
    arr = tensor.detach().mul(255).add_(0.5).clamp_(0, 255).permute(1, 2, 0).to("cpu", torch.uint8).numpy()
    Image.fromarray(arr).save(path)


class FusionInterpolator:

    def __init__(self, adacof_model, fusion_net, phase_net_state=None, device=None):
        self.adacof = adacof_model
        self.fusion_net = fusion_net
        self.device = torch.device(device) if device is not None else next(fusion_net.parameters()).device
        self.phase_net_state = phase_net_state
        self._per_size = {}
        import inspect
        net = getattr(adacof_model, "model", adacof_model)
        self._adacof_kwargs = {"return_sides": False} if "return_sides" in inspect.signature(net.forward).parameters else {}

    def _state(self, h, w):
        key = (h, w)
        if key not in self._per_size:
            height = calc_pyr_height(torch.empty(3, h, w, device="meta"))
            pyr = Pyramid(height=height, nbands=4, scale_factor=np.sqrt(2), device=self.device)
            pyr.set_full_size(h, w)
            net = PhaseNet(pyr, self.device, num_img=2)
            if self.phase_net_state is not None:
                net.load_state_dict(self.phase_net_state)
            net.eval()
            self._per_size[key] = (pyr, net)
        return self._per_size[key]

    @torch.no_grad()
    def __call__(self, rgb_frame1, rgb_frame2, output_baseline=False):
        h, w = rgb_frame1.shape[1:]
        pyr, phase_net = self._state(h, w)
        nlev = pyr.height - 2
        lab12 = torch.empty((6, h, w), dtype=torch.float32, device=rgb_frame1.device)
        ops.rgb2lab(rgb_frame1, out=lab12[:3])
        ops.rgb2lab(rgb_frame2, out=lab12[3:])
        f1, f2 = rgb_frame1.unsqueeze(0), rgb_frame2.unsqueeze(0)
        return self._run(rgb_frame1, rgb_frame2, output_baseline, pyr, phase_net, nlev, lab12, f1, f2)

    def _run(self, rgb_frame1, rgb_frame2, output_baseline, pyr, phase_net, nlev, lab12, f1, f2):
        h, w = rgb_frame1.shape[1:]
        vals, bufs, amp_max = pyr.filter(lab12, concat_frames=2, phase_scale=1.0 / math.pi,
                                         amp_max_eps=phase_net.eps)
        vals_pred = phase_net(phase_net.normalize_vals(vals, concat=bufs, amp_max=amp_max))
        lab_pred = pyr.inv_filter(DecompValues(0, vals_pred.phase, vals_pred.amplitude, vals_pred.low_level))
        phase_pred = ops.lab2rgb(lab_pred)
        pp = phase_pred.unsqueeze(0)

        _, _, three, masks = self.adacof(torch.cat((f1, f1, pp), 0), torch.cat((f2, pp, f2), 0), **self._adacof_kwargs)
        ada_pred, flow_var_map, between = three[:1], masks[:1], three[1:]

        coarse = min(6, nlev)
        m = ops.channel_mean_diff(ada_pred, phase_pred.unsqueeze(0), 1.0, False, signed=True)
        hf = pyr.band_filter(m, level_mask=1, keep_high=True)
        maps = torch.empty((1, 3, h, w), dtype=torch.float32, device=rgb_frame1.device)
        d = ops.absdiff(hf, None, 100.0, True)
        phase_uncertainty = ops.gaussian_filter(d, 5, out=maps[:, 1])
        mask = ((1 << coarse) - 1) << (nlev - coarse)
        vb = pyr.filter(torch.cat((ada_pred[0], phase_pred), 0), level_mask=mask, want_high=False)
        half = lambda t: (t[:12], t[12:])
        dp, da = [0] * nlev, [0] * nlev
        for k in range(nlev - coarse, nlev):
            dp[k] = ops.absdiff(*half(vb.phase[k])[::-1])
            da[k] = ops.absdiff(*half(vb.amplitude[k])[::-1])
        dlow = ops.absdiff(vb.low_level[3:], vb.low_level[:3])
        freq = pyr.inv_filter(DecompValues(0, dp, da, dlow))
        fd = ops.channel_mean_diff(freq.unsqueeze(0), None, 30.0, False)
        ada_uncertainty = ops.absdiff(fd, ops.median_filter(fd, 50), 5.0, True, out=maps[:, 0])

        _, _, base, _ = self.adacof(between[:1], between[1:], **self._adacof_kwargs)

        out = {"phase_pred": pp, "ada_pred": ada_pred, "base": base, "flow_var_map": flow_var_map,
               "phase_uncertainty": phase_uncertainty, "ada_uncertainty": ada_uncertainty}
        if output_baseline:
            split = nlev // 2
            fine = (1 << split) - 1
            lab = pyr.band_filter_pair(ops.rgb2lab(ada_pred[0]), dict(level_mask=((1 << nlev) - 1) & ~fine, keep_high=True),
                                       ops.rgb2lab(phase_pred), dict(level_mask=fine, keep_low=True))
            out["baseline"] = ops.lab2rgb(lab).unsqueeze(0)

        other = lab12.unsqueeze(0)
        maps[:, 2].copy_(flow_var_map[:, 0])
        out["final"] = self.fusion_net(base, ada_pred, pp, other, maps, variant=0)
        return out


def build_models(args, device):
    if getattr(args, "loaded_adacof_model", None) is not None:
        adacof_model = args.loaded_adacof_model
    else:
        adacof_model = Model(SimpleNamespace(gpu_id=args.gpu_id, model=getattr(args, "adacof_model", DEFAULT_ADACOF_MODEL),
                                             kernel_size=args.adacof_kernel_size, dilation=args.adacof_dilation,
                                             config=getattr(args, "adacof_config", None)))
        adacof_model.eval()
        ckpt = getattr(args, "adacof_checkpoint", None)
        if ckpt and os.path.exists(ckpt):
            adacof_model.load(torch.load(ckpt, map_location="cpu")["state_dict"])
    if getattr(args, "loaded_fusion_net", None) is not None:
        fusion_net = args.loaded_fusion_net
    else:
        fusion_net = FusionNet().to(device)
        fusion_net.load_state_dict(torch.load(args.checkpoint, map_location="cpu"))
        fusion_net.eval()
    return adacof_model, fusion_net


_INTERPOLATORS = {}
_MAX_INTERPOLATORS = 4


def _interpolator_for(args, device):
    pn = getattr(args, "phase_net_checkpoint", "./src/phase_net/phase_net.pt")
    if getattr(args, "loaded_adacof_model", None) is not None and getattr(args, "loaded_fusion_net", None) is not None:
        key = ("loaded", id(args.loaded_adacof_model), id(args.loaded_fusion_net), pn, device.index)
    else:
        key = ("files", getattr(args, "adacof_model", DEFAULT_ADACOF_MODEL), getattr(args, "adacof_checkpoint", None),
# ... 31 lines not shown
```

### fusion-method-for-video-frame-interpolation_amd/vfi_amd/ops.py

```python
import os

import torch

from . import _lib
from ._lib import VfiLibraryError

ACT = {None: 0, "none": 0, "relu": 1, "elu": 2, "tanh": 3, "sigmoid": 4}
PAD = {"zeros": 0, "zero": 0, "reflect": 1}


def _slice_ptr(t, name):
    if not isinstance(t, torch.Tensor) or not t.is_cuda:
        raise VfiLibraryError(f"{name} must be a tensor on a HIP device (vfi_amd has no CPU path)")
    if t.dtype != torch.float32 or t.dim() != 4:
        raise VfiLibraryError(f"{name} must be a 4-d float32 tensor")
    _lib.check_device(t, name)
    n, c, h, w = t.shape
    sn, sc, sh, sw = t.stride()
    if not ((sw == 1 or w == 1) and (sh == w or h == 1) and (sc == h * w or c == 1)):
        raise VfiLibraryError(f"{name}: per-sample (C,H,W) block must be dense, strides {t.stride()}")
    if n == 1:
        sn = c * h * w
    return t.data_ptr(), sn


def new(shape, like):
    return torch.empty(shape, dtype=torch.float32, device=like.device)


class PackedConv:

    def __init__(self, weight, bias=None, bn=None, device=None):
        device = torch.device(device) if device is not None else weight.device
        if device.type != "cuda":
            raise VfiLibraryError("PackedConv needs a HIP device (vfi_amd has no CPU path)")
        weight = weight.detach().to(device=device, dtype=torch.float32).contiguous()
        self.cout, self.cin, kh, kw = weight.shape
        assert kh == kw, "square kernels only"
        self.ks = kh
        cout = self.cout
        b = (bias.detach().to(device=device, dtype=torch.float32) if bias is not None
             else torch.zeros(cout, device=device))
        scale = None
        if bn is not None:
            g, beta, mean, var, eps = bn
            f = lambda t: t.detach().to(device=device, dtype=torch.float32)
            scale = (f(g) / torch.sqrt(f(var) + eps)).contiguous()
            b = (b - f(mean)) * scale + f(beta)
        self.bias = b.contiguous()
        n = _lib.lib().vfi_conv2d_packed_floats(cout, self.cin, self.ks)
        if n <= 0:
            raise VfiLibraryError(f"vfi_conv2d_packed_floats rejected {tuple(weight.shape)}")
        self.packed = torch.empty(n, dtype=torch.float32, device=device)
        _lib.call("vfi_conv2d_pack", weight.data_ptr(), scale.data_ptr() if scale is not None else None,
                  self.packed.data_ptr(), cout, self.cin, self.ks, _lib.stream_ptr())
        self._keep = (weight, scale)


WINOGRAD = os.environ.get("VFI_CONV_WINOGRAD", "1") != "0"
FUSED_RESIZE = (not WINOGRAD) or os.environ.get("VFI_CONV_FUSED_RESIZE", "0") == "1"
def _winograd_work(n, cin, cout, h, w, residual=False, pooled=False, act="relu"):
    algo = _lib.lib().vfi_conv2d_algo(n, cin, h, w, cout, 3, int(bool(residual)), int(bool(pooled)), ACT[act])
    if algo == 2:
        name = "conv3x3_winograd4_kernel" if os.environ.get("VFI_CONV_WINOGRAD4M", "1") == "0" else "conv3x3_winograd4m_kernel"
        return ("flop", 2.0 * n * cin * cout * 36 * (h * w / 16.0), name)
    if algo == 1:
        return ("flop", 2.0 * n * cin * cout * 16 * (h * w / 4.0), "conv3x3_winograd_kernel")
    return ("flop", 2.0 * n * cin * cout * 9 * h * w, "conv2d_mfma_kernel<3,8,%d>" % (2 if ((cout + 31) // 32 * 32) % 64 == 0 else 1))


_WORKSPACES = {}
WORKSPACE_FLOATS = 48 * 1024 * 1024


def _workspace(device):
    key = (device.index, torch.cuda.current_stream(device).cuda_stream)
    ws = _WORKSPACES.get(key)
    if ws is None:
        ws = _WORKSPACES[key] = torch.empty(WORKSPACE_FLOATS, dtype=torch.float32, device=device)
    return ws


def conv2d(x, pc, pad_mode="zeros", act=None, residual=None, out=None, upsample2x=False):
    n, cin, h, w = x.shape
    if cin != pc.cin:
        raise VfiLibraryError(f"conv2d: input has {cin} channels, weights expect {pc.cin}")
    if upsample2x and pc.ks == 3 and not FUSED_RESIZE:
        x = resize_bilinear(x, (2 * h, 2 * w), align_corners=True)
        h, w, upsample2x = 2 * h, 2 * w, False
    if upsample2x:
        h, w = 2 * h, 2 * w
    if out is None:
        out = new((n, pc.cout, h, w), x)
    elif tuple(out.shape) != (n, pc.cout, h, w):
        raise VfiLibraryError(f"conv2d: out shape {tuple(out.shape)} != {(n, pc.cout, h, w)}")
    xp, xs = _slice_ptr(x, "x")
    yp, ys = _slice_ptr(out, "out")
    rp, rs = (None, 0)
    if residual is not None:
        if tuple(residual.shape) != tuple(out.shape):
            raise VfiLibraryError("conv2d: residual shape mismatch")
        rp, rs = _slice_ptr(residual, "residual")
    ws = _workspace(x.device)
    work = None
    if _lib.PROFILE is not None:
        if pc.ks == 3 and not upsample2x and WINOGRAD:
            work = _winograd_work(n, cin, pc.cout, h, w, residual is not None, False, act)
        else:
            label = (f"conv2d_mfma_kernel<{pc.ks},{4 if pc.ks == 5 else 8},{2 if ((pc.cout + 31) // 32 * 32) % 64 == 0 else 1}"
                     + (",ups>" if upsample2x else ">"))
            work = ("flop", 2.0 * n * cin * pc.cout * pc.ks * pc.ks * h * w, label)
            if pc.ks == 1:
                if _lib.lib().vfi_conv2d_algo(n, cin, h, w, pc.cout, 1, int(residual is not None), 0, ACT[act]) == 3:
                    label = "conv1x1_stream_kernel"
                work = ("byte", 4.0 * n * (cin + pc.cout) * h * w, label)
    _lib.call("vfi_conv2d_upsample2x" if upsample2x else "vfi_conv2d", xp, xs, pc.packed.data_ptr(), pc.bias.data_ptr(), rp, rs, yp, ys,
              n, cin, h, w, pc.cout, pc.ks, PAD[pad_mode], ACT[act], ws.data_ptr(), ws.numel(), _lib.stream_ptr(), work=work)
    return out


def conv2d_pool2(x, pc, is_max, pad_mode="zeros", act="relu"):
    n, cin, h, w = x.shape
    if cin != pc.cin:
        raise VfiLibraryError(f"conv2d_pool2: input has {cin} channels, weights expect {pc.cin}")
    out, pooled = new((n, pc.cout, h, w), x), new((n, pc.cout, h // 2, w // 2), x)
    xp, xs = _slice_ptr(x, "x")
    ws = _workspace(x.device)
    work = None
    if _lib.PROFILE is not None:
        if pc.ks == 3 and WINOGRAD:
            work = _winograd_work(n, cin, pc.cout, h, w, False, True, act)
        else:
            work = ("flop", 2.0 * n * cin * pc.cout * pc.ks * pc.ks * h * w,
                    f"conv2d_mfma_kernel<{pc.ks},{4 if pc.ks == 5 else 8},{2 if ((pc.cout + 31) // 32 * 32) % 64 == 0 else 1}>")
    _lib.call("vfi_conv2d_pool2", xp, xs, pc.packed.data_ptr(), pc.bias.data_ptr(), out.data_ptr(), out.stride(0),
              pooled.data_ptr(), pooled.stride(0), int(bool(is_max)), n, cin, h, w, pc.cout, pc.ks, PAD[pad_mode], ACT[act],
              ws.data_ptr(), ws.numel(), _lib.stream_ptr(), work=work)
    return out, pooled


def conv2d_resized_prefix(x, x2, pc, pad_mode="reflect", act=None, out=None):
    n, cin, h, w = x.shape
    n2, c2, hs, ws_ = x2.shape
    if cin != pc.cin or n2 != n:
        raise VfiLibraryError("conv2d_resized_prefix: shape mismatch")
    if pc.ks == 3 and not FUSED_RESIZE:
        resize_bilinear(x2, (h, w), align_corners=False, out=x[:, :c2])
        return conv2d(x, pc, pad_mode=pad_mode, act=act, out=out)
    if out is None:
        out = new((n, pc.cout, h, w), x)
    xp, xs = _slice_ptr(x, "x")
    x2p, x2s = _slice_ptr(x2, "x2")
    yp, ys = _slice_ptr(out, "out")
    ws = _workspace(x.device)
    work = None
    if _lib.PROFILE is not None:
        work = ("flop", 2.0 * n * cin * pc.cout * pc.ks * pc.ks * h * w, f"conv2d_mfma_kernel<{pc.ks},8,2,rsz>")
    _lib.call("vfi_conv2d_resized_prefix", xp, xs, x2p, x2s, c2, hs, ws_, pc.packed.data_ptr(), pc.bias.data_ptr(), yp, ys,
              n, cin, h, w, pc.cout, pc.ks, PAD[pad_mode], ACT[act], ws.data_ptr(), ws.numel(), _lib.stream_ptr(), work=work)
    return out


def adacof_prepare(frame0, frame2, rgbx=True):
    n, c, h, w = frame0.shape
    if c != 3 or tuple(frame2.shape) != tuple(frame0.shape):
        raise VfiLibraryError("adacof_prepare: frames must both be (N,3,H,W)")
    hp, wp = (h + 31) // 32 * 32, (w + 31) // 32 * 32
    shape = (n, hp, wp, 4) if rgbx else (n, 3, hp, wp)
    pad0, pad2, x6 = new(shape, frame0), new(shape, frame0), new((n, 6, hp, wp), frame0)
    _lib.call("vfi_adacof_prepare", _lib.dptr(frame0, "frame0"), _lib.dptr(frame2, "frame2"), pad0.data_ptr(),
              pad2.data_ptr(), x6.data_ptr(), n, h, w, hp, wp, int(bool(rgbx)), _lib.stream_ptr())
    return pad0, pad2, x6


def pool2(x, is_max, out=None):
    n, c, h, w = x.shape
    if out is None:
        out = new((n, c, h // 2, w // 2), x)
    xp, xs = _slice_ptr(x, "x")
    yp, ys = _slice_ptr(out, "out")
    _lib.call("vfi_pool2", xp, xs, yp, ys, n, c, h, w, int(bool(is_max)), _lib.stream_ptr())
    return out


def resize_bilinear(x, size, align_corners, relu_input=False, residual=None, out=None):
    n, c, h, w = x.shape
    ho, wo = size
    if out is None:
        out = new((n, c, ho, wo), x)
    xp, xs = _slice_ptr(x, "x")
    yp, ys = _slice_ptr(out, "out")
    rp, rs = (None, 0) if residual is None else _slice_ptr(residual, "residual")
    _lib.call("vfi_resize_bilinear", xp, xs, rp, rs, yp, ys, n, c, h, w, ho, wo, int(bool(align_corners)),
              int(bool(relu_input)), _lib.stream_ptr())
    return out

# ... 921 lines not shown
        raise VfiLibraryError("l1_forward: shape mismatch")
    out = new((1,), a)
    _lib.call("vfi_l1_forward", _lib.dptr(a, "a"), _lib.dptr(b, "b"), a.numel(), int(bool(wrap)), float(scale),
              _reduce_workspace(a).data_ptr(), out.data_ptr(), _lib.stream_ptr(),
              work=_prof("byte", 8.0 * a.numel(), "l1_forward"))
    return out[0]


def l1_backward(a, b, upstream, wrap=False, scale=1.0, need_a=True, need_b=True):
    ga = torch.empty_like(a) if need_a else None
    gb = torch.empty_like(b) if need_b else None
    _lib.call("vfi_l1_backward", _lib.dptr(a, "a"), _lib.dptr(b, "b"), _lib.dptr(upstream.reshape(1), "upstream"),
              _lib.dptr(ga), _lib.dptr(gb), a.numel(), int(bool(wrap)), float(scale), _lib.stream_ptr(),
              work=_prof("byte", 4.0 * a.numel() * (2 + need_a + need_b), "l1_backward"))
    return ga, gb


def _out_like(x, out, name):
    if out is None:
        return torch.empty_like(x)
    if tuple(out.shape) != tuple(x.shape) or not out.is_contiguous() or out.dtype != torch.float32 or out.device != x.device:
        raise VfiLibraryError(f"{name}: out must be a contiguous float32 tensor of shape {tuple(x.shape)} on {x.device}")
    return out


def rgb2lab(rgb, out=None):
    x = rgb.contiguous()
    hw = x.shape[-1] * x.shape[-2]
    out = _out_like(x, out, "rgb2lab")
    _lib.call("vfi_rgb2lab", _lib.dptr(x, "rgb"), out.data_ptr(), x.numel() // (3 * hw), hw, _lib.stream_ptr())
    return out


def lab2rgb(lab):
    x = lab.contiguous()
    hw = x.shape[-1] * x.shape[-2]
    out = torch.empty_like(x)
    _lib.call("vfi_lab2rgb", _lib.dptr(x, "lab"), out.data_ptr(), x.numel() // (3 * hw), hw, _lib.stream_ptr())
    return out


def channel_mean_diff(a, b=None, scale=1.0, clamp01=False, signed=False):
    a = a.contiguous()
    n, c, h, w = a.shape
    out = torch.empty((n, h, w), dtype=torch.float32, device=a.device)
    _lib.call("vfi_channel_mean_diff", _lib.dptr(a, "a"), _lib.dptr(b.contiguous(), "b") if b is not None else None,
              out.data_ptr(), n, c, h * w, float(scale), int(bool(clamp01)) | (2 if signed else 0), _lib.stream_ptr())
    return out


def absdiff(x, y, scale=1.0, clamp01=False, out=None):
    x = x.contiguous()
    if y is not None:
        y = y.contiguous()
        if x.shape != y.shape:
            raise VfiLibraryError("absdiff: shape mismatch")
    out = _out_like(x, out, "absdiff")
    _lib.call("vfi_absdiff", _lib.dptr(x, "x"), _lib.dptr(y, "y") if y is not None else None, out.data_ptr(), x.numel(),
              float(scale), int(bool(clamp01)), _lib.stream_ptr())
    return out


def gaussian_filter(x, sigma, truncate=4.0, out=None):
    x = x.contiguous()
    n, h, w = x.shape
    tmp, out = torch.empty_like(x), _out_like(x, out, "gaussian_filter")
    _lib.call("vfi_gaussian_filter", _lib.dptr(x, "x"), tmp.data_ptr(), out.data_ptr(), n, h, w, float(sigma),
              float(truncate), _lib.stream_ptr())
    return out

# ... 54 lines not shown
```

### fusion-method-for-video-frame-interpolation_amd/vfi_amd/phase_net/phase_net.py

```python
import math
import os

import torch

from .. import _lib, ops
from ..nn_util import BatchNormParams, ConvParams, Indexed, PackedModule
from ..values import DecompValues, NormalizedValues


class PhaseNetBlock(torch.nn.Module):

    def __init__(self, c_in, c_out, pred_out, kernel_size, device=None, dropout=0.5):
        super().__init__()
        k = kernel_size[0]
        self.feature_map = Indexed({0: ConvParams(c_in, c_out, k), 1: BatchNormParams(c_out),
                                    3: ConvParams(c_out, c_out, k)})
        self.prediction_map = Indexed({0: ConvParams(c_out, pred_out, 1)})
        self.batch_stats = False
        self.train(False)
        if device is not None:
            self.to(device)

    def batch_statistics(self, mode=True):
        self.batch_stats = bool(mode)
# ... 147 lines not shown
        high = torch.zeros((hs[0], 1, hs[2], hs[3]), dtype=torch.float32, device=low_in.device)

        concat = getattr(vals, "concat", None)

        def level_input(idx):
            if concat is not None:
                return concat[idx]
            ph, am = vals.phase[idx], vals.amplitude[idx]
            _, c, h, w = ph.shape
            p_prev = p_low if idx == 0 else p_band
            x = ops.new((b, 64 + p_prev + 2 * c, h, w), low_in)
            ops.affine_slice(ph.contiguous(), x[:, 64 + p_prev:64 + p_prev + c])
            ops.affine_slice(am.contiguous(), x[:, 64 + p_prev + c:])
            return x

        def layer(idx):
            return idx + 1 if idx + 1 < len(self.layers) - 1 else len(self.layers) - 1

        tail_env = os.environ.get("VFI_PHASENET_TAIL", "")
        tail_on = n_img == 2 and not ops.FUSED_RESIZE and tail_env != "0"
        tail_min = 0 if tail_env == "1" else ops.PHASENET_TAIL_MIN_PIXELS
        phases, amps = [], []
        x_next = None
        for idx in range(m):
            p_prev = p_low if idx == 0 else p_band
            _, c, h, w = vals.phase[idx].shape
            filled = x_next is not None
            x = x_next if filled else level_input(idx)
            i = layer(idx)
            fused = packed[i][0].ks == 3 and (64 + p_prev) % 8 == 0
            if not fused and not filled:
                ops.resize_bilinear(fp, (h, w), align_corners=False, out=x[:, :64 + p_prev])
            tail = tail_on and idx + 1 < m and h * w >= tail_min and packed[layer(idx + 1)][0].ks == 3 and (64 + p_band) % 8 == 0
            fp = block(i, x, ops.new((b, 64 if tail else 64 + p_band, h, w), low_in), prev=fp if fused and not filled else None, head=False)
            amp_in = x[:, 64 + p_prev + c:]
            cp = packed[i][2]
            if cp.cout != p_band or cp.ks != 1:
                raise RuntimeError(f"PhaseNet: a band level's prediction map must be a 1x1 layer with {p_band} outputs (phase_net.py:23-35)")
            x_next = None
            if tail:
                x_next = level_input(idx + 1)
                p_out, a_out = ops.phasenet_level_tail(fp, cp, amp_in, self.max_amplitudes[idx], x_next[:, :64 + p_band])
            elif n_img == 2:
                p_out, a_out = ops.new((b * 4, 1, h, w), low_in), ops.new((b * 4, 1, h, w), low_in)
                _lib.call("vfi_phasenet_predict", fp.data_ptr(), fp.stride(0), cp.packed.data_ptr(), cp.bias.data_ptr(), amp_in.data_ptr(),
                          x.stride(0), self.max_amplitudes[idx].data_ptr(), fp[:, 64:].data_ptr(), fp.stride(0), p_out.data_ptr(),
                          a_out.data_ptr(), b, 64, h, w, stream,
                          work=("byte", 4.0 * b * (64 + 8 + 8 + 8) * h * w, "phasenet_predict_kernel") if _lib.PROFILE is not None else None)
            else:
                if c != 4 * n_img:
                    raise RuntimeError(f"PhaseNet(num_img={n_img}): level {idx} has {c} phase planes, expected {4 * n_img}")
                _, p_out, a_out = ops.phasenet_predict_n(fp[:, :64], cp, amp_in, self.max_amplitudes[idx], n_img, pred=fp[:, 64:])
            phases.append(p_out); amps.append(a_out)
        for _ in range(self.pyr.height - 2 - m):
            phases.append(0); amps.append(0)
        return DecompValues(high, phases[::-1], amps[::-1], low)

    def _forward_grad(self, vals, m):
        from . import grad as G
        n_img = self.num_img
        low_in = vals.low_level.detach().contiguous()
        if low_in.shape[1] != n_img:
            raise RuntimeError(f"PhaseNet(num_img={n_img}): the low level has {low_in.shape[1]} images")
        f, c = G.block_forward(self.layers[0], low_in)
        low = G.blend_low(c, low_in, self.max_low_level, n_img)
        hs = vals.high_level.shape
        high = torch.zeros((hs[0], 1, hs[2], hs[3]), dtype=torch.float32, device=low_in.device)
        phases, amps = [], []
        for idx in range(m):
            ph, am = vals.phase[idx].detach(), vals.amplitude[idx].detach()
            i = idx + 1 if idx + 1 < len(self.layers) - 1 else len(self.layers) - 1
            blk = self.layers[i]
            if ph.shape[1] != 4 * n_img:
                raise RuntimeError(f"PhaseNet(num_img={n_img}): level {idx} has {ph.shape[1]} phase planes, expected {4 * n_img}")
            x = G.level_input(f, c, ph, am)
            f = G.block_features(blk, x)
            c, p_out, a_out = G.level_head(blk, f, am, self.max_amplitudes[idx], n_img)
            phases.append(p_out); amps.append(a_out)
        for _ in range(self.pyr.height - 2 - m):
            phases.append(0); amps.append(0)
        return DecompValues(high, phases[::-1], amps[::-1], low)
# ... 1 lines not shown
```

### include/vfi_hip.h

```cpp
#ifndef VFI_HIP_H
#define VFI_HIP_H

#include <stddef.h>
#include <stdint.h>

#ifdef __cplusplus
extern "C" {
#endif

#define VFI_ABI_VERSION 1

typedef void *vfi_stream_t;

typedef enum vfi_status {
    VFI_OK = 0,
    VFI_ERR_INVALID_ARG = -1,
    VFI_ERR_SHAPE = -2,
    VFI_ERR_LAUNCH = -3,
    VFI_ERR_UNSUPPORTED = -4,
    VFI_ERR_FFT = -5,
    VFI_ERR_NOMEM = -6
} vfi_status;

int vfi_abi_version(void);
const char *vfi_status_string(int status);
const char *vfi_last_error(void);
int vfi_debug_poison_lds(vfi_stream_t stream);
int vfi_debug_conv_override(int winograd4_mode, int max_workgroups);


int vfi_adacof_forward(const float *input, const float *weight, const float *offset_i,
                       const float *offset_j, float *output, int N, int C, int Hin, int Win,
                       int H, int W, int F, int dilation, vfi_stream_t stream);

int vfi_adacof_backward(const float *grad_output, const float *input, const float *weight,
                        const float *offset_i, const float *offset_j,
                        float *grad_weight, float *grad_offset_i, float *grad_offset_j,
                        int N, int C, int Hin, int Win, int H, int W, int F, int dilation,
                        vfi_stream_t stream);

int vfi_adacof_fused(const float *frame0, const float *frame2,
                     const float *w1, const float *a1, const float *b1,
                     const float *w2, const float *a2, const float *b2, const float *occ,
                     float *out_t1, float *out_t2, float *out_frame, float *out_mask,
                     int N, int C, int H, int W, int F, int dilation, vfi_stream_t stream);

int vfi_adacof_fused_rgbx(const float *frame0_rgbx, const float *frame2_rgbx,
                          const float *w1, const float *a1, const float *b1,
                          const float *w2, const float *a2, const float *b2, const float *occ,
                          float *out_t1, float *out_t2, float *out_frame, float *out_mask,
                          int N, int H, int W, int F, int dilation, int weights_are_logits, vfi_stream_t stream);


typedef enum vfi_act {
    VFI_ACT_NONE = 0,
    VFI_ACT_RELU = 1,
    VFI_ACT_ELU = 2,
    VFI_ACT_TANH = 3,
    VFI_ACT_SIGMOID = 4
} vfi_act;

typedef enum vfi_pad { VFI_PAD_ZERO = 0, VFI_PAD_REFLECT = 1 } vfi_pad;

long long vfi_conv2d_packed_floats(int Cout, int Cin, int KS);

int vfi_conv2d_pack(const float *w_oihw, const float *scale, float *packed, int Cout, int Cin, int KS,
                    vfi_stream_t stream);

enum { VFI_CONV_ALGO_DIRECT = 0, VFI_CONV_ALGO_WINOGRAD2 = 1, VFI_CONV_ALGO_WINOGRAD4 = 2, VFI_CONV_ALGO_STREAM1X1 = 3 };
int vfi_conv2d_algo(int N, int Cin, int H, int W, int Cout, int KS, int has_residual, int pooled, int act);

int vfi_conv2d(const float *x, long long x_bstride, const float *packed_w, const float *bias,
               const float *residual, long long res_bstride, float *y, long long y_bstride, int N, int Cin,
               int H, int W, int Cout, int KS, int pad_mode, int act, float *workspace,
               long long workspace_floats, vfi_stream_t stream);

int vfi_conv2d_pool2(const float *x, long long x_bstride, const float *packed_w, const float *bias, float *y,
                     long long y_bstride, float *pooled, long long pooled_bstride, int is_max, int N, int Cin, int H, int W,
                     int Cout, int KS, int pad_mode, int act, float *workspace, long long workspace_floats,
                     vfi_stream_t stream);

int vfi_conv2d_upsample2x(const float *x_lowres, long long x_bstride, const float *packed_w, const float *bias,
                          const float *residual, long long res_bstride, float *y, long long y_bstride, int N,
                          int Cin, int H, int W, int Cout, int KS, int pad_mode, int act, float *workspace,
                          long long workspace_floats, vfi_stream_t stream);

int vfi_conv2d_resized_prefix(const float *x, long long x_bstride, const float *x2, long long x2_bstride,
                              int prefix_channels, int Hs, int Ws, const float *packed_w, const float *bias,
                              float *y, long long y_bstride, int N, int Cin, int H, int W, int Cout, int KS,
                              int pad_mode, int act, float *workspace, long long workspace_floats,
                              vfi_stream_t stream);


int vfi_adacof_prepare(const float *frame0, const float *frame2, float *pad0, float *pad2, float *x6, int N,
                       int H, int W, int Hp, int Wp, int rgbx, vfi_stream_t stream);

int vfi_pool2(const float *x, long long x_bstride, float *y, long long y_bstride, int N, int C, int H, int W,
              int is_max, vfi_stream_t stream);

int vfi_resize_bilinear(const float *x, long long x_bstride, const float *residual, long long res_bstride,
                        float *y, long long y_bstride, int N, int C, int Hin, int Win, int Hout, int Wout,
                        int align_corners, int relu_input, vfi_stream_t stream);

int vfi_upsample2x_tapsum(const float *taps_lowres, float *out, int N, int Hs, int Ws, float bias, int act,
                          vfi_stream_t stream);

int vfi_softmax_channels(const float *x, long long x_bstride, float *y, long long y_bstride, int N, int C, int HW,
                         vfi_stream_t stream);

int vfi_affine_slice(const float *src, long long src_bstride, float *dst, long long dst_bstride, int N,
                     long long count, const float *div_per_sample, float mul, vfi_stream_t stream);

int vfi_batch_max(const float *x, long long x_bstride, int N, long long count, float eps, float *out_max,
                  void *workspace_u32, vfi_stream_t stream);

int vfi_phasenet_emit(const float *pred, long long pred_bstride, const float *amp_in, long long amp_bstride,
                      const float *max_amp, float *phase_out, float *amp_out, int N, int HW, vfi_stream_t stream);

int vfi_phasenet_predict(const float *feat, long long feat_bstride, const float *packed_w, const float *bias,
                         const float *amp_in, long long amp_bstride, const float *max_amp, float *pred, long long pred_bstride,
                         float *phase_out, float *amp_out, int N, int Cin, int H, int W, vfi_stream_t stream);

int vfi_phasenet_level_tail(const float *feat, long long feat_bstride, const float *packed_w, const float *bias,
                            const float *amp_in, long long amp_bstride, const float *max_amp, float *x_next,
                            long long next_bstride, float *phase_out, float *amp_out, int N, int H, int W, int Hout, int Wout,
                            vfi_stream_t stream);

int vfi_phasenet_emit_low(const float *pred, long long pred_bstride, const float *low_in, long long low_bstride,
                          const float *max_low, float *low_out, int N, int HW, vfi_stream_t stream);
// ... 275 lines not shown
```

Before: 25.95 frames/s.

## Write fused AdaCoF output directly into cropped per-sample buffers and skip dead stores

Adds a cropped-destination variant of the fused AdaCoF kernel that writes the blended frame and mask straight into per-sample assembled buffers, and limits the grid to the crop. It also adds a pointer-array prepare kernel that reads per-sample frames without stacking, lets conv+pool skip the full-resolution output when only the pooled result is needed, and lets PhaseNet's top-level predict skip storing predictions. The aim is to remove intermediate copies, crops and unneeded full-resolution writes at 1080p, at the cost of more kernel variants and env-gated paths.

```diff
diff --git a/fusion-method-for-video-frame-interpolation_amd/csrc/vfi_adacof.hip b/fusion-method-for-video-frame-interpolation_amd/csrc/vfi_adacof.hip
--- a/fusion-method-for-video-frame-interpolation_amd/csrc/vfi_adacof.hip
+++ b/fusion-method-for-video-frame-interpolation_amd/csrc/vfi_adacof.hip
@@ -156,13 +156,20 @@
     float m, q;
 };
 
-template <int C, int VEC, int FT, int UNROLL_L, int MIN_WAVES, bool RGBX = false, bool SOFTMAX = false, bool WIN = false>
+struct FusedDst {
+    float *frame[VFI_MAX_SAMPLE_PTRS], *mask[VFI_MAX_SAMPLE_PTRS];
+    long long frame_cstride;
+    int h0, w0;
+};
+
+template <int C, int VEC, int FT, int UNROLL_L, int MIN_WAVES, bool RGBX = false, bool SOFTMAX = false, bool WIN = false, bool CROP = false>
 __global__ __launch_bounds__(256, MIN_WAVES) void adacof_fused_kernel(
     const float *__restrict__ frame0, const float *__restrict__ frame2,
     const float *__restrict__ w1, const float *__restrict__ a1, const float *__restrict__ b1,
     const float *__restrict__ w2, const float *__restrict__ a2, const float *__restrict__ b2,
     const float *__restrict__ occ, float *__restrict__ out_t1, float *__restrict__ out_t2,
-    float *__restrict__ out_frame, float *__restrict__ out_mask, int H, int W, int Frt, int dil, int margin) {
+    float *__restrict__ out_frame, float *__restrict__ out_mask, int H, int W, int Frt, int dil, int margin, const FusedDst dst) {
+    static_assert(!CROP || VEC == 1, "the cropped destination is written pixel by pixel");
     const int F = FT > 0 ? FT : Frt;
     const int x0 = (blockIdx.x * 64 + threadIdx.x) * VEC;
     const int y = blockIdx.y * 4 + threadIdx.y;
@@ -341,6 +348,22 @@
 
     Vec<VEC> o;
     o.load(occ + (size_t)n * plane + pix);
+    if constexpr (CROP) {
+        if (y >= dst.h0 || x0 >= dst.w0) return;
+        const size_t cpix = (size_t)y * dst.w0 + x0;
+        float *__restrict__ fo = dst.frame[n] + cpix;
+#pragma unroll
+        for (int c = 0; c < C; ++c) {
+#pragma clang fp contract(off)
+            const float t1 = res[0][0][c], t2 = res[1][0][c];
+            fo[(size_t)c * dst.frame_cstride] = o.v[0] * t1 + (1.0f - o.v[0]) * t2;
+        }
+        if (float *mo = dst.mask[n]) {
+            const float mx = fmaxf(var[0][0], var[1][0]);
+            mo[cpix] = fminf(fmaxf(mx, 0.0f), 20.0f) / 20.0f;
+        }
+        return;
+    }
 #pragma unroll
     for (int c = 0; c < C; ++c) {
         const size_t q = ((size_t)n * C + c) * plane + pix;
@@ -511,8 +534,8 @@
                              const float *a1, const float *b1, const float *w2, const float *a2,
                              const float *b2, const float *occ, float *out_t1, float *out_t2,
                              float *out_frame, float *out_mask, int N, int C, int H, int W, int F,
-                             int dilation, bool rgbx, bool softmax, vfi_stream_t stream) {
-    VFI_REQUIRE(frame0 && frame2 && w1 && a1 && b1 && w2 && a2 && b2 && occ && out_frame,
+                             int dilation, bool rgbx, bool softmax, vfi_stream_t stream, const FusedDst *crop = nullptr) {
+    VFI_REQUIRE(frame0 && frame2 && w1 && a1 && b1 && w2 && a2 && b2 && occ && (out_frame || crop),
                 VFI_ERR_INVALID_ARG, "vfi_adacof_fused: null pointer");
     VFI_REQUIRE(N > 0 && H > 0 && W > 0 && F > 0 && dilation > 0, VFI_ERR_INVALID_ARG,
                 "vfi_adacof_fused: non-positive size");
@@ -533,35 +556,45 @@
     if (rgbx) VFI_REQUIRE(aligned16(frame0) && aligned16(frame2), VFI_ERR_INVALID_ARG, "vfi_adacof_fused_rgbx: frames must be 16-B aligned");
     hipStream_t s = vfi::as_stream(stream);
     dim3 block(64, 4);
-    dim3 grid(vfi::ceil_div(W, 64 * vec), vfi::ceil_div(H, 4), N);
+    dim3 grid(vfi::ceil_div(crop ? crop->w0 : W, 64 * vec), vfi::ceil_div(crop ? crop->h0 : H, 4), N);
     VFI_REQUIRE(grid.z <= 65535 && grid.y <= 65535, VFI_ERR_UNSUPPORTED, "vfi_adacof_fused: grid too large");
 #define LAUNCH(VEC, FT, UN, MW)                                                                          \
     hipLaunchKernelGGL((adacof_fused_kernel<3, VEC, FT, UN, MW>), grid, block, 0, s, frame0, frame2, w1, a1, b1, \
-                       w2, a2, b2, occ, out_t1, out_t2, out_frame, out_mask, H, W, F, dilation, 0)
+                       w2, a2, b2, occ, out_t1, out_t2, out_frame, out_mask, H, W, F, dilation, 0, FusedDst{})
     if (softmax) VFI_REQUIRE(rgbx, VFI_ERR_UNSUPPORTED, "vfi_adacof_fused: softmax folding needs the rgbx entry point");
     static const int win_margin = getenv("VFI_ADACOF_MARGIN") ? atoi(getenv("VFI_ADACOF_MARGIN")) : 4;
     const int wh = 4 + (F - 1) * dilation + 2 * win_margin + 1, ww = 64 + (F - 1) * dilation + 2 * win_margin + 1;
     const size_t win_bytes = 2ull * wh * ww * sizeof(float4);
+    if (crop) {
+        VFI_REQUIRE(rgbx && softmax && win_margin > 0 && win_bytes <= 64 * 1024, VFI_ERR_UNSUPPORTED,
+                    "vfi_adacof_fused_rgbx_crop: needs logits and an LDS-window kernel ((F-1)*dilation <= 10, VFI_ADACOF_MARGIN > 0)");
+#define LAUNCH_CROP(FT, UN)                                                                                                \
+    hipLaunchKernelGGL((adacof_fused_kernel<3, 1, FT, UN, 3, true, true, true, true>), grid, block, win_bytes, s, frame0, frame2, w1, \
+                       a1, b1, w2, a2, b2, occ, nullptr, nullptr, nullptr, nullptr, H, W, F, dilation, win_margin, *crop)
+        if (F == 5) LAUNCH_CROP(5, 5); else LAUNCH_CROP(0, 1);
+#undef LAUNCH_CROP
+        return vfi::check_launch("vfi_adacof_fused_rgbx_crop");
+    }
     if (rgbx && win_margin > 0 && win_bytes <= 64 * 1024) {
 #define LAUNCH_WIN(FT, UN, SM)                                                                                       \
     hipLaunchKernelGGL((adacof_fused_kernel<3, 1, FT, UN, 3, true, SM, true>), grid, block, win_bytes, s, frame0, frame2, w1, \
-                       a1, b1, w2, a2, b2, occ, out_t1, out_t2, out_frame, out_mask, H, W, F, dilation, win_margin)
+                       a1, b1, w2, a2, b2, occ, out_t1, out_t2, out_frame, out_mask, H, W, F, dilation, win_margin, FusedDst{})
         if (F == 5) { if (softmax) LAUNCH_WIN(5, 5, true); else LAUNCH_WIN(5, 5, false); }
         else        { if (softmax) LAUNCH_WIN(0, 1, true); else LAUNCH_WIN(0, 1, false); }
 #undef LAUNCH_WIN
     } else if (rgbx) {
         if (F == 5 && softmax)
             hipLaunchKernelGGL((adacof_fused_kernel<3, 1, 5, 5, 3, true, true>), grid, block, 0, s, frame0, frame2, w1, a1, b1,
-                               w2, a2, b2, occ, out_t1, out_t2, out_frame, out_mask, H, W, F, dilation, 0);
+                               w2, a2, b2, occ, out_t1, out_t2, out_frame, out_mask, H, W, F, dilation, 0, FusedDst{});
         else if (softmax)
             hipLaunchKernelGGL((adacof_fused_kernel<3, 1, 0, 1, 4, true, true>), grid, block, 0, s, frame0, frame2, w1, a1, b1,
-                               w2, a2, b2, occ, out_t1, out_t2, out_frame, out_mask, H, W, F, dilation, 0);
+                               w2, a2, b2, occ, out_t1, out_t2, out_frame, out_mask, H, W, F, dilation, 0, FusedDst{});
         else if (F == 5)
             hipLaunchKernelGGL((adacof_fused_kernel<3, 1, 5, 5, 3, true>), grid, block, 0, s, frame0, frame2, w1, a1, b1,
-                               w2, a2, b2, occ, out_t1, out_t2, out_frame, out_mask, H, W, F, dilation, 0);
+                               w2, a2, b2, occ, out_t1, out_t2, out_frame, out_mask, H, W, F, dilation, 0, FusedDst{});
         else
             hipLaunchKernelGGL((adacof_fused_kernel<3, 1, 0, 1, 4, true>), grid, block, 0, s, frame0, frame2, w1, a1, b1,
-                               w2, a2, b2, occ, out_t1, out_t2, out_frame, out_mask, H, W, F, dilation, 0);
+                               w2, a2, b2, occ, out_t1, out_t2, out_frame, out_mask, H, W, F, dilation, 0, FusedDst{});
     } else if (F == 5) {
         if (vec == 4) LAUNCH(4, 5, 1, 3);
         else if (vec == 2) LAUNCH(2, 5, 1, 4);
@@ -590,3 +623,24 @@
     return adacof_fused_impl(frame0_rgbx, frame2_rgbx, w1, a1, b1, w2, a2, b2, occ, out_t1, out_t2, out_frame,
                              out_mask, N, 3, H, W, F, dilation, true, weights_are_logits != 0, stream);
 }
+
+extern "C" int vfi_adacof_fused_rgbx_crop(const float *frame0_rgbx, const float *frame2_rgbx, const float *w1, const float *a1,
+                                          const float *b1, const float *w2, const float *a2, const float *b2, const float *occ,
+                                          float *const *out_frames, long long frame_cstride, float *const *out_masks, int N, int H,
+                                          int W, int h0, int w0, int F, int dilation, vfi_stream_t stream) {
+    VFI_REQUIRE(out_frames, VFI_ERR_INVALID_ARG, "vfi_adacof_fused_rgbx_crop: null pointer");
+    VFI_REQUIRE(N > 0 && N <= VFI_MAX_SAMPLE_PTRS, VFI_ERR_UNSUPPORTED, "vfi_adacof_fused_rgbx_crop: %d samples (1 to %d)", N, VFI_MAX_SAMPLE_PTRS);
+    VFI_REQUIRE(h0 > 0 && w0 > 0 && h0 <= H && w0 <= W && frame_cstride >= (long long)h0 * w0, VFI_ERR_INVALID_ARG,
+                "vfi_adacof_fused_rgbx_crop: crop %dx%d of %dx%d, channel stride %lld", h0, w0, H, W, frame_cstride);
+    FusedDst dst{};
+    for (int n = 0; n < N; ++n) {
+        VFI_REQUIRE(out_frames[n], VFI_ERR_INVALID_ARG, "vfi_adacof_fused_rgbx_crop: null frame destination of sample %d", n);
+        dst.frame[n] = out_frames[n];
+        dst.mask[n] = out_masks ? out_masks[n] : nullptr;
+    }
+    dst.frame_cstride = frame_cstride;
+    dst.h0 = h0;
+    dst.w0 = w0;
+    return adacof_fused_impl(frame0_rgbx, frame2_rgbx, w1, a1, b1, w2, a2, b2, occ, nullptr, nullptr, nullptr, nullptr, N, 3, H, W, F,
+                             dilation, true, true, stream, &dst);
+}
diff --git a/fusion-method-for-video-frame-interpolation_amd/csrc/vfi_aux.hip b/fusion-method-for-video-frame-interpolation_amd/csrc/vfi_aux.hip
--- a/fusion-method-for-video-frame-interpolation_amd/csrc/vfi_aux.hip
+++ b/fusion-method-for-video-frame-interpolation_amd/csrc/vfi_aux.hip
@@ -21,6 +21,33 @@
         } else {
             p0[i] = a;
             p2[i] = b;
+        }
+        x6[((size_t)n * 6 + c) * plane + pix] = a - mean;
+        x6[((size_t)n * 6 + 3 + c) * plane + pix] = b - mean;
+    }
+}
+
+struct PrepareFrames {
+    const float *f0[VFI_MAX_SAMPLE_PTRS], *f2[VFI_MAX_SAMPLE_PTRS];
+};
+__global__ void adacof_prepare_ptrs_kernel(const PrepareFrames fr, float *__restrict__ p0, float *__restrict__ p2,
+                                           float *__restrict__ x6, int H, int W, int Hp, int Wp, int rgbx) {
+    const int n = blockIdx.y;
+    const float *__restrict__ f0 = fr.f0[n], *__restrict__ f2 = fr.f2[n];
+    const int total = 3 * Hp * Wp;
+    for (int i = blockIdx.x * blockDim.x + threadIdx.x; i < total; i += gridDim.x * blockDim.x) {
+        const int x = i % Wp, y = (i / Wp) % Hp, c = i / (Wp * Hp);
+        const int sy = y < H ? y : 2 * (H - 1) - y, sx = x < W ? x : 2 * (W - 1) - x;
+        const size_t s = ((size_t)c * H + sy) * W + sx;
+        const float mean = c == 0 ? 0.4631f : (c == 1 ? 0.4352f : 0.3990f);
+        const float a = f0[s], b = f2[s];
+        const size_t plane = (size_t)Hp * Wp, pix = (size_t)y * Wp + x;
+        if (rgbx) {
+            p0[((size_t)n * plane + pix) * 4 + c] = a;
+            p2[((size_t)n * plane + pix) * 4 + c] = b;
+        } else {
+            p0[(size_t)n * 3 * plane + i] = a;
+            p2[(size_t)n * 3 * plane + i] = b;
         }
         x6[((size_t)n * 6 + c) * plane + pix] = a - mean;
         x6[((size_t)n * 6 + 3 + c) * plane + pix] = b - mean;
@@ -349,6 +376,26 @@
     return vfi::check_launch("vfi_adacof_prepare");
 }
 
+extern "C" int vfi_adacof_prepare_ptrs(const float *const *frames0, const float *const *frames2, float *pad0, float *pad2, float *x6,
+                                       int N, int H, int W, int Hp, int Wp, int rgbx, vfi_stream_t stream) {
+    VFI_REQUIRE(frames0 && frames2 && pad0 && pad2 && x6, VFI_ERR_INVALID_ARG, "vfi_adacof_prepare_ptrs: null pointer");
+    VFI_REQUIRE(N > 0 && N <= VFI_MAX_SAMPLE_PTRS, VFI_ERR_UNSUPPORTED, "vfi_adacof_prepare_ptrs: %d samples (1 to %d)", N, VFI_MAX_SAMPLE_PTRS);
+    VFI_REQUIRE(H > 0 && W > 0 && Hp >= H && Wp >= W, VFI_ERR_INVALID_ARG, "vfi_adacof_prepare_ptrs: bad sizes");
+    VFI_REQUIRE(Hp - H < H && Wp - W < W, VFI_ERR_SHAPE, "vfi_adacof_prepare_ptrs: reflect pad %dx%d needs a larger frame than %dx%d",
+                Hp - H, Wp - W, H, W);
+    VFI_REQUIRE(3ll * Hp * Wp < (1ll << 31), VFI_ERR_UNSUPPORTED, "vfi_adacof_prepare_ptrs: frame too large");
+    PrepareFrames fr{};
+    for (int n = 0; n < N; ++n) {
+        VFI_REQUIRE(frames0[n] && frames2[n], VFI_ERR_INVALID_ARG, "vfi_adacof_prepare_ptrs: null frame of sample %d", n);
+        fr.f0[n] = frames0[n];
+        fr.f2[n] = frames2[n];
+    }
+    const long long per_sample = 3ll * Hp * Wp;
+    hipLaunchKernelGGL(adacof_prepare_ptrs_kernel, dim3(vfi::blocks_1d(per_sample), (unsigned)N), dim3(kThreads), 0, vfi::as_stream(stream),
+                       fr, pad0, pad2, x6, H, W, Hp, Wp, rgbx);
+    return vfi::check_launch("vfi_adacof_prepare_ptrs");
+}
+
 extern "C" int vfi_pool2(const float *x, long long x_bstride, float *y, long long y_bstride, int N, int C, int H,
                          int W, int is_max, vfi_stream_t stream) {
     VFI_REQUIRE(x && y, VFI_ERR_INVALID_ARG, "vfi_pool2: null pointer");
diff --git a/fusion-method-for-video-frame-interpolation_amd/csrc/vfi_conv.hip b/fusion-method-for-video-frame-interpolation_amd/csrc/vfi_conv.hip
--- a/fusion-method-for-video-frame-interpolation_amd/csrc/vfi_conv.hip
+++ b/fusion-method-for-video-frame-interpolation_amd/csrc/vfi_conv.hip
@@ -406,7 +406,7 @@
     return vfi::check_launch("vfi_conv2d");
 }
 
-template <int VEC>
+template <int VEC, bool PRED = true>
 __global__ __launch_bounds__(256) void phasenet_predict_kernel(const float *__restrict__ x, long long x_bs, const float *__restrict__ wp,
                                                                const float *__restrict__ bias, int Cout_pad, const float *__restrict__ amp_in,
                                                                long long amp_bs, const float *__restrict__ maxv, float *__restrict__ pred,
@@ -449,14 +449,14 @@
             for (int k = 0; k < VEC; ++k) acc[o][k] = fmaf(wo, v[k], acc[o][k]);
         }
     }
-    vec *pp = reinterpret_cast<vec *>(pred + (size_t)n * pred_bs) + q;
+    vec *pp = PRED ? reinterpret_cast<vec *>(pred + (size_t)n * pred_bs) + q : nullptr;
 #pragma unroll
     for (int o = 0; o < 8; ++o) {
         const float b = bias ? bias[o] : 0.0f;
         vec r;
 #pragma unroll
         for (int k = 0; k < VEC; ++k) r[k] = acc[o][k] = apply_act(acc[o][k] + b, 3);
-        pp[(size_t)o * plane] = r;
+        if (PRED) pp[(size_t)o * plane] = r;
     }
     const vec *ap = reinterpret_cast<const vec *>(amp_in + (size_t)n * amp_bs) + q;
     vec *pho = reinterpret_cast<vec *>(phase_out + (size_t)n * 4 * HW) + q, *amo = reinterpret_cast<vec *>(amp_out + (size_t)n * 4 * HW) + q;
@@ -593,7 +593,7 @@
                        long long workspace_floats, vfi_stream_t stream, const float *x2 = nullptr, long long x2_bstride = 0,
                        int rsz_channels = 0, int Hs = 0, int Ws = 0, float *pooled = nullptr, long long pooled_bstride = 0,
                        int pool_max = 0) {
-    VFI_REQUIRE(x && packed_w && y, VFI_ERR_INVALID_ARG, "vfi_conv2d: null pointer");
+    VFI_REQUIRE(x && packed_w && (y || (pooled && !ups && !x2)), VFI_ERR_INVALID_ARG, "vfi_conv2d: null pointer");
     VFI_REQUIRE(N > 0 && Cin > 0 && Cout > 0 && H > 0 && W > 0, VFI_ERR_INVALID_ARG, "vfi_conv2d: non-positive size");
     VFI_REQUIRE(KS == 1 || KS == 3 || KS == 5, VFI_ERR_UNSUPPORTED, "vfi_conv2d: kernel size %d", KS);
     VFI_REQUIRE(pad_mode == 0 || pad_mode == 1, VFI_ERR_INVALID_ARG, "vfi_conv2d: pad_mode %d", pad_mode);
@@ -643,6 +643,7 @@
         return launch_winograd(a, N, s);
     }
     if (pooled) {
+        VFI_REQUIRE(y, VFI_ERR_UNSUPPORTED, "vfi_conv2d_pool2: a null full-resolution output needs a 3x3 layer on the Winograd path");
         const int rc = conv2d_impl(x, x_bstride, packed_w, bias, residual, res_bstride, y, y_bstride, N, Cin, H, W, Cout, KS, pad_mode,
                                    act, false, workspace, workspace_floats, stream);
         return rc ? rc : vfi_pool2(y, y_bstride, pooled, pooled_bstride, N, Cout, H, W, pool_max, stream);
@@ -689,23 +690,31 @@
 extern "C" int vfi_phasenet_predict(const float *feat, long long feat_bstride, const float *packed_w, const float *bias,
                                     const float *amp_in, long long amp_bstride, const float *max_amp, float *pred, long long pred_bstride,
                                     float *phase_out, float *amp_out, int N, int Cin, int H, int W, vfi_stream_t stream) {
-    VFI_REQUIRE(feat && packed_w && amp_in && max_amp && pred && phase_out && amp_out, VFI_ERR_INVALID_ARG, "vfi_phasenet_predict: null pointer");
+    VFI_REQUIRE(feat && packed_w && amp_in && max_amp && phase_out && amp_out, VFI_ERR_INVALID_ARG, "vfi_phasenet_predict: null pointer");
     VFI_REQUIRE(N > 0 && N <= 65535 && Cin > 0 && H > 0 && W > 0, VFI_ERR_INVALID_ARG, "vfi_phasenet_predict: bad sizes");
     const long long HW = (long long)H * W;
     VFI_REQUIRE((long long)Cin * HW < (1ll << 31), VFI_ERR_UNSUPPORTED, "vfi_phasenet_predict: per-sample tensor too large for 32-bit offsets");
     ConvArgs a{};
-    a.x = feat; a.y = pred; a.x_bs = feat_bstride; a.y_bs = pred_bstride; a.Cout = 8; a.H = H; a.W = W;
+    a.x = feat; a.y = pred; a.x_bs = feat_bstride; a.y_bs = pred ? pred_bstride : 0; a.Cout = 8; a.H = H; a.W = W;
     int vec = conv1x1_stream_vec(a, 1);
     const uintptr_t bits = reinterpret_cast<uintptr_t>(amp_in) | reinterpret_cast<uintptr_t>(phase_out) | reinterpret_cast<uintptr_t>(amp_out) | (uintptr_t)(amp_bstride * 4);
     if (vec == 4 && (bits & 15u)) vec = (bits & 7u) ? 0 : 2;
     else if (vec == 2 && (bits & 7u)) vec = 0;
     if (!vec) {
+        VFI_REQUIRE(pred, VFI_ERR_UNSUPPORTED, "vfi_phasenet_predict: a null prediction map needs the streaming kernel (>= 4096 pixels, an even count, aligned planes)");
         const int rc = conv2d_impl(feat, feat_bstride, packed_w, bias, nullptr, 0, pred, pred_bstride, N, Cin, H, W, 8, 1, 0, 3, false, nullptr, 0, stream);
         return rc ? rc : vfi_phasenet_emit(pred, pred_bstride, amp_in, amp_bstride, max_amp, phase_out, amp_out, N, (int)HW, stream);
     }
     const dim3 grid((unsigned)vfi::ceil_div((int)(HW / vec), 256), (unsigned)N);
     hipStream_t s = vfi::as_stream(stream);
-    if (vec == 4)
+    if (!pred) {
+        if (vec == 4)
+            hipLaunchKernelGGL((phasenet_predict_kernel<4, false>), grid, dim3(256), 0, s, feat, feat_bstride, packed_w, bias, 32, amp_in, amp_bstride, max_amp,
+                               pred, 0, phase_out, amp_out, Cin, (int)HW);
+        else
+            hipLaunchKernelGGL((phasenet_predict_kernel<2, false>), grid, dim3(256), 0, s, feat, feat_bstride, packed_w, bias, 32, amp_in, amp_bstride, max_amp,
+                               pred, 0, phase_out, amp_out, Cin, (int)HW);
+    } else if (vec == 4)
         hipLaunchKernelGGL(phasenet_predict_kernel<4>, grid, dim3(256), 0, s, feat, feat_bstride, packed_w, bias, 32, amp_in, amp_bstride, max_amp, pred,
                            pred_bstride, phase_out, amp_out, Cin, (int)HW);
     else
diff --git a/fusion-method-for-video-frame-interpolation_amd/csrc/vfi_conv_winograd.hip b/fusion-method-for-video-frame-interpolation_amd/csrc/vfi_conv_winograd.hip
--- a/fusion-method-for-video-frame-interpolation_amd/csrc/vfi_conv_winograd.hip
+++ b/fusion-method-for-video-frame-interpolation_amd/csrc/vfi_conv_winograd.hip
@@ -251,6 +251,7 @@
             const float *__restrict__ resp = (RES && !split_out && a.res) ? a.res + (size_t)it.n * a.res_bs : nullptr;
             float *__restrict__ yp = split_out ? a.ws + ((size_t)it.split * N + it.n) * a.Cout * HW : a.y + (size_t)it.n * a.y_bs;
             const int act = ACT >= 0 ? ACT : (split_out ? 0 : a.act);
+            const bool store_y = !POOL || a.y;
             const int co0 = it.nb * T::BN + 4 * k4;
             const float *bias_l = lds + T::BIAS_OFF + (cseq & (T::BIAS_SLOTS - 1)) * 64 + 4 * k4;
             auto outputs = [&](int mb, int j, float2 (&o)[2]) {
@@ -292,7 +293,7 @@
                         const float b = split_out ? 0.0f : bias_l[dc];
                         q.x = apply_act(q.x + b, act); q.y = apply_act(q.y + b, act);
                         q.z = apply_act(q.z + b, act); q.w = apply_act(q.w + b, act);
-                        if (co0 + dc < a.Cout) {
+                        if (store_y && co0 + dc < a.Cout) {
                             if (RES && resp) {
                                 const float4 r = *reinterpret_cast<const float4 *>(resp + off + (size_t)dc * HW);
                                 q.x += r.x; q.y += r.y; q.z += r.z; q.w += r.w;
@@ -314,7 +315,7 @@
                         if (POOL && pool_ok) pq[(size_t)dc * Hq * Wq] = pooled(o, b);
 #pragma unroll
                         for (int dy = 0; dy < 2; ++dy)
-                            if (gy0 + dy < a.H) {
+                            if (store_y && gy0 + dy < a.H) {
                                 const size_t e = off + (size_t)dc * HW + (size_t)dy * a.W;
                                 float vx = apply_act(o[dy].x + b, act), vy = apply_act(o[dy].y + b, act);
                                 if (RES && resp) {
@@ -415,6 +416,8 @@
     dim3 grid(capped_grid(items < resident ? items : resident));
     const int act = b.splits > 1 ? 0 : b.act;
     const bool pool_fused = b.pool && b.splits == 1 && !b.res && act == 1;
+    if (!b.y && !pool_fused)
+        return vfi::fail(VFI_ERR_UNSUPPORTED, "vfi_conv2d_pool2: a null full-resolution output needs the pooled epilogue (a plain ReLU layer in one K split)");
     if (pool_fused) {
         hipLaunchKernelGGL((conv3x3_winograd_kernel<false, 1, true>), grid, dim3(256), T::LDS_BYTES, s, b);
         return vfi::check_launch("vfi_conv2d");
diff --git a/fusion-method-for-video-frame-interpolation_amd/csrc/vfi_conv_winograd4.hip b/fusion-method-for-video-frame-interpolation_amd/csrc/vfi_conv_winograd4.hip
--- a/fusion-method-for-video-frame-interpolation_amd/csrc/vfi_conv_winograd4.hip
+++ b/fusion-method-for-video-frame-interpolation_amd/csrc/vfi_conv_winograd4.hip
@@ -255,7 +255,7 @@
                                 for (int c = 0; c < 4; ++c) prev[c] = o[c];
                             }
                         }
-                        if (gy < a.H) {
+                        if ((!POOL || a.y) && gy < a.H) {
                             if (vec4) {
                                 if (gx < a.W) {
                                     float4 q = make_float4(o[0], o[1], o[2], o[3]);
diff --git a/fusion-method-for-video-frame-interpolation_amd/csrc/vfi_conv_winograd4m.hip b/fusion-method-for-video-frame-interpolation_amd/csrc/vfi_conv_winograd4m.hip
--- a/fusion-method-for-video-frame-interpolation_amd/csrc/vfi_conv_winograd4m.hip
+++ b/fusion-method-for-video-frame-interpolation_amd/csrc/vfi_conv_winograd4m.hip
@@ -91,7 +91,7 @@
 #define W4M_STAMP(var)
 #endif
 
-template <int ACT, bool RES = false, bool POOL = false>
+template <int ACT, bool RES = false, int POOL = 0>
 __global__ __launch_bounds__(256, 1) void conv3x3_winograd4m_kernel(const ConvArgs a) {
     using T = Wino4Tile;
     extern __shared__ __attribute__((aligned(16))) float lds[];
@@ -283,7 +283,7 @@
         const int gx = it.x0 + 4 * n16, gy0 = it.y0 + 4 * wave;
         const int act = ACT >= 0 ? ACT : a.act;
         const unsigned plane_bytes = (unsigned)HW * 4u, row_bytes = (unsigned)a.W * 4u;
-        const __amdgpu_buffer_rsrc_t ydesc = make_rsrc(a.y + (size_t)it.n * a.y_bs, (unsigned)a.Cout * plane_bytes);
+        const __amdgpu_buffer_rsrc_t ydesc = make_rsrc(POOL == 2 ? a.pool : a.y + (size_t)it.n * a.y_bs, POOL == 2 ? 0u : (unsigned)a.Cout * plane_bytes);
         const __amdgpu_buffer_rsrc_t rdesc = make_rsrc(RES ? a.res + (size_t)it.n * a.res_bs : a.y, RES ? (unsigned)a.Cout * plane_bytes : 0u);
         const int Hq = a.H >> 1, Wq = a.W >> 1;
         const __amdgpu_buffer_rsrc_t pdesc = make_rsrc(POOL ? a.pool + (size_t)it.n * a.pool_bs : a.y, POOL ? (unsigned)a.Cout * (unsigned)(Hq * Wq) * 4u : 0u);
@@ -381,7 +381,7 @@
                         for (int c = 0; c < 4; ++c) prev[c] = o[c];
                     }
                 }
-                if (FAST || gy0 + r < a.H) {
+                if (POOL != 2 && (FAST || gy0 + r < a.H)) {
                     const int soff = (int)(r * row_bytes);
                     if (row4) {
                         if (RES) {
@@ -519,7 +519,8 @@
                               reinterpret_cast<const void *>(conv3x3_winograd4m_kernel<2>), reinterpret_cast<const void *>(conv3x3_winograd4m_kernel<3>),
                               reinterpret_cast<const void *>(conv3x3_winograd4m_kernel<4>), reinterpret_cast<const void *>(conv3x3_winograd4m_kernel<-1, true>),
                               reinterpret_cast<const void *>(conv3x3_winograd4m_kernel<1, true>),
-                              reinterpret_cast<const void *>(conv3x3_winograd4m_kernel<1, false, true>)})
+                              reinterpret_cast<const void *>(conv3x3_winograd4m_kernel<1, false, 1>),
+                              reinterpret_cast<const void *>(conv3x3_winograd4m_kernel<1, false, 2>)})
             if (e == hipSuccess) e = hipFuncSetAttribute(k, hipFuncAttributeMaxDynamicSharedMemorySize, (int)W4M::LDS_BYTES);
         int dev = 0, cus = 0;
         if (e == hipSuccess) e = hipGetDevice(&dev);
@@ -529,7 +530,8 @@
     }
     dim3 grid(capped_grid(b.wino_items < resident ? b.wino_items : resident));
     const size_t lds = W4M::LDS_BYTES;
-    if (b.pool) hipLaunchKernelGGL((conv3x3_winograd4m_kernel<1, false, true>), grid, dim3(W4M::THREADS), lds, s, b);
+    if (b.pool && !b.y) hipLaunchKernelGGL((conv3x3_winograd4m_kernel<1, false, 2>), grid, dim3(W4M::THREADS), lds, s, b);
+    else if (b.pool) hipLaunchKernelGGL((conv3x3_winograd4m_kernel<1, false, 1>), grid, dim3(W4M::THREADS), lds, s, b);
     else if (b.res && b.act == 1) hipLaunchKernelGGL((conv3x3_winograd4m_kernel<1, true>), grid, dim3(W4M::THREADS), lds, s, b);
     else if (b.res) hipLaunchKernelGGL((conv3x3_winograd4m_kernel<-1, true>), grid, dim3(W4M::THREADS), lds, s, b);
     else if (b.act == 0) hipLaunchKernelGGL((conv3x3_winograd4m_kernel<0>), grid, dim3(W4M::THREADS), lds, s, b);
diff --git a/fusion-method-for-video-frame-interpolation_amd/vfi_amd/_lib.py b/fusion-method-for-video-frame-interpolation_amd/vfi_amd/_lib.py
--- a/fusion-method-for-video-frame-interpolation_amd/vfi_amd/_lib.py
+++ b/fusion-method-for-video-frame-interpolation_amd/vfi_amd/_lib.py
@@ -23,6 +23,8 @@
     "vfi_adacof_forward": [c_f] * 5 + [c_i] * 8 + [c_s],
     "vfi_adacof_backward": [c_f] * 8 + [c_i] * 8 + [c_s],
     "vfi_adacof_fused": [c_f] * 13 + [c_i] * 6 + [c_s],
+    "vfi_adacof_fused_rgbx_crop": [c_f] * 9 + [c_f, c_l, c_f] + [c_i] * 7 + [c_s],
+    "vfi_adacof_prepare_ptrs": [c_f] * 5 + [c_i] * 6 + [c_s],
     "vfi_conv2d_packed_floats": [c_i] * 3,
     "vfi_conv2d_algo": [c_i] * 9,
     "vfi_conv2d_pack": [c_f] * 3 + [c_i] * 3 + [c_s],
diff --git a/fusion-method-for-video-frame-interpolation_amd/vfi_amd/adacof/cupy_module/adacof.py b/fusion-method-for-video-frame-interpolation_amd/vfi_amd/adacof/cupy_module/adacof.py
--- a/fusion-method-for-video-frame-interpolation_amd/vfi_amd/adacof/cupy_module/adacof.py
+++ b/fusion-method-for-video-frame-interpolation_amd/vfi_amd/adacof/cupy_module/adacof.py
@@ -1,3 +1,4 @@
+import ctypes
 import math
 
 import torch
@@ -57,6 +58,30 @@
     return grad_weight, grad_offset_i, grad_offset_j
 
 
+def adacof_fused_crop(frame0, frame2, w1, a1, b1, w2, a2, b2, occ, dilation, frames_out, masks_out=None):
+    from ... import ops
+    n, hp, wp = frame0.shape[0], frame0.shape[1], frame0.shape[2]
+    f = int(math.sqrt(w1.size(1)))
+    masks_out = list(masks_out) if masks_out is not None else [None] * n
+    if len(frames_out) != n or len(masks_out) != n:
+        raise _lib.VfiLibraryError("adacof_fused_crop: one destination per sample")
+    h0, w0 = (int(v) for v in frames_out[0].shape[-2:])
+    views = [t.reshape(3, h0, w0) if t.dim() == 4 else t for t in frames_out]
+    cs = views[0].stride(0)
+    for t in views:
+        if not t.is_cuda or t.dtype != torch.float32 or tuple(t.shape) != (3, h0, w0) or t.stride() != (cs, w0, 1):
+            raise _lib.VfiLibraryError("adacof_fused_crop: frame destinations must be float32 (3,h0,w0) with dense planes and one channel stride")
+    for m in masks_out:
+        if m is not None and (not m.is_cuda or m.dtype != torch.float32 or m.numel() != h0 * w0 or not m.is_contiguous()):
+            raise _lib.VfiLibraryError("adacof_fused_crop: a mask destination must be a dense float32 tensor of h0*w0 elements")
+    fp, mp = ops.sample_ptrs(views), ops.sample_ptrs(masks_out)
+    d = _lib.dptr
+    n_masks = sum(m is not None for m in masks_out)
+    _lib.call("vfi_adacof_fused_rgbx_crop", d(frame0, "frame0"), d(frame2, "frame2"), d(w1), d(a1), d(b1), d(w2), d(a2), d(b2), d(occ),
+              ctypes.addressof(fp), cs, ctypes.addressof(mp) if n_masks else None, n, hp, wp, h0, w0, f, int(dilation), _lib.stream_ptr(),
+              work=("byte", float(n) * h0 * w0 * (6 * f * f * 4 + 4 + 2 * 4 * 3 + 4 * 3) + 4.0 * n_masks * h0 * w0, "adacof_fused_kernel"))
+
+
 def adacof_fused(frame0, frame2, w1, a1, b1, w2, a2, b2, occ, dilation,
                  want_sides=True, want_mask=True, rgbx=False, weights_are_logits=False):
     if rgbx:
diff --git a/fusion-method-for-video-frame-interpolation_amd/vfi_amd/fusion_net/fusion_adacofnet.py b/fusion-method-for-video-frame-interpolation_amd/vfi_amd/fusion_net/fusion_adacofnet.py
--- a/fusion-method-for-video-frame-interpolation_amd/vfi_amd/fusion_net/fusion_adacofnet.py
+++ b/fusion-method-for-video-frame-interpolation_amd/vfi_amd/fusion_net/fusion_adacofnet.py
@@ -3,7 +3,7 @@
 import torch
 
 from .. import _lib, ops
-from ..adacof.cupy_module.adacof import FunctionAdaCoF, adacof_fused
+from ..adacof.cupy_module.adacof import FunctionAdaCoF, adacof_fused, adacof_fused_crop
 from ..nn_util import ConvParams, Indexed, PackedModule
 
 HEADS = ("moduleWeight1", "moduleAlpha1", "moduleBeta1", "moduleWeight2", "moduleAlpha2", "moduleBeta2",
@@ -67,10 +67,10 @@
             x = ops.conv2d(x, pc, "zeros", "relu")
         return x
 
-    def _basic_pooled(self, convs, x):
+    def _basic_pooled(self, convs, x, pooled_only=False):
         for pc in convs[:-1]:
             x = ops.conv2d(x, pc, "zeros", "relu")
-        return ops.conv2d_pool2(x, convs[-1], False, "zeros", "relu")
+        return ops.conv2d_pool2(x, convs[-1], False, "zeros", "relu", pooled_only=pooled_only)
 
     def _up(self, pc, x, skip):
         return ops.conv2d(x, pc, "zeros", "relu", residual=skip, upsample2x=True)
@@ -79,7 +79,7 @@
         if softmax and self.wants_graph():
             return _KernelEstimationFunction.apply(self, x6, *self.parameters())
         p = self.packed()
-        c1, q1 = self._basic_pooled(p["moduleConv1"], x6)
+        _, q1 = self._basic_pooled(p["moduleConv1"], x6, pooled_only=ops.lean_frame())
         c2, q2 = self._basic_pooled(p["moduleConv2"], q1)
         c3, q3 = self._basic_pooled(p["moduleConv3"], q2)
         c4, q4 = self._basic_pooled(p["moduleConv4"], q3)
@@ -282,7 +282,16 @@
             raise NotImplementedError("vfi_amd implements the inference path only (eval mode)")
         return super().train(False)
 
-    def forward(self, frame0, frame2, return_sides=True):
+    def forward(self, frame0, frame2, return_sides=True, frames_out=None, masks_out=None):
+        if frames_out is not None:
+            if return_sides:
+                raise ValueError("AdaCoFNet.forward: frames_out needs return_sides=False")
+            if any(tuple(a.shape) != tuple(b.shape) for a, b in zip(frame0, frame2)):
+                sys.exit("Frame sizes do not match")
+            pad0, pad2, x6 = ops.adacof_prepare([t.contiguous() for t in frame0], [t.contiguous() for t in frame2], rgbx=True)
+            w1, a1, b1, w2, a2, b2, occ = self.get_kernel.forward_x6(x6, softmax=False)
+            adacof_fused_crop(pad0, pad2, w1, a1, b1, w2, a2, b2, occ, self.dilation, frames_out, masks_out)
+            return None, None, frames_out, masks_out
         h0, w0 = int(frame0.shape[2]), int(frame0.shape[3])
         if h0 != int(frame2.shape[2]) or w0 != int(frame2.shape[3]):
             sys.exit("Frame sizes do not match")
diff --git a/fusion-method-for-video-frame-interpolation_amd/vfi_amd/fusion_net/fusion_net.py b/fusion-method-for-video-frame-interpolation_amd/vfi_amd/fusion_net/fusion_net.py
--- a/fusion-method-for-video-frame-interpolation_amd/vfi_amd/fusion_net/fusion_net.py
+++ b/fusion-method-for-video-frame-interpolation_amd/vfi_amd/fusion_net/fusion_net.py
@@ -38,28 +38,37 @@
     def train(self, mode=True):
         return torch.nn.Module.train(self, mode)
 
-    def forward(self, base, adacof, phase, other, maps, save=False, variant=0):
+    def forward(self, base, adacof, phase, other, maps, save=False, variant=0, assembled=None):
         params = [t for c in self._live_convs() for t in (c.weight, c.bias)]
         inputs = [base, adacof, phase, other, maps]
         if torch.is_grad_enabled() and (any(t is not None and t.requires_grad for t in inputs) or
                                         (self.training and any(t.requires_grad for t in params))):
             out = _FusionNetFunction.apply(self, variant, *inputs, *params)
         else:
-            out = self._forward_impl(self.packed(), base, adacof, phase, other, maps, variant, None)
+            out = self._forward_impl(self.packed(), base, adacof, phase, other, maps, variant, None, assembled)
         if save:
             self.residuals.append(float((out - (phase if variant == 1 else base)).sum().item()))
         return out
 
-    def _forward_impl(self, p, base, adacof, phase, other, maps, variant, keep):
+    def _forward_impl(self, p, base, adacof, phase, other, maps, variant, keep, assembled=None):
         parts = [base, adacof, phase, other] + ([maps] if maps is not None else [])
         n, _, h, w = base.shape
         if h % 8 or w % 8:
             raise ops.VfiLibraryError(f"FusionNet needs H, W multiples of 8, got {h}x{w}")
-        x = ops.new((n, self.in_channels, h, w), base)
-        c0 = 0
-        for t in parts:
-            ops.affine_slice(t.contiguous(), x[:, c0:c0 + t.shape[1]])
-            c0 += t.shape[1]
+        if assembled is not None:
+            x, c0 = assembled, 0
+            for t in parts:
+                s = assembled[:, c0:c0 + t.shape[1]]
+                same = all(a == b for size, a, b in zip(s.shape, t.stride(), s.stride()) if size > 1)
+                if t.data_ptr() != s.data_ptr() or tuple(t.shape) != tuple(s.shape) or not same:
+                    raise ops.VfiLibraryError("FusionNet: `assembled` must hold base, adacof, phase, other, maps as its channel slices")
+                c0 += t.shape[1]
+        else:
+            x = ops.new((n, self.in_channels, h, w), base)
+            c0 = 0
+            for t in parts:
+                ops.affine_slice(t.contiguous(), x[:, c0:c0 + t.shape[1]])
+                c0 += t.shape[1]
         assert c0 == self.in_channels
         enc_in, skip = [x], []
         for i in range(3):
diff --git a/fusion-method-for-video-frame-interpolation_amd/vfi_amd/fusion_net/interpolate_twoframe.py b/fusion-method-for-video-frame-interpolation_amd/vfi_amd/fusion_net/interpolate_twoframe.py
--- a/fusion-method-for-video-frame-interpolation_amd/vfi_amd/fusion_net/interpolate_twoframe.py
+++ b/fusion-method-for-video-frame-interpolation_amd/vfi_amd/fusion_net/interpolate_twoframe.py
@@ -39,7 +39,8 @@
         self._per_size = {}
         import inspect
         net = getattr(adacof_model, "model", adacof_model)
-        self._adacof_kwargs = {"return_sides": False} if "return_sides" in inspect.signature(net.forward).parameters else {}
+        self._adacof_params = inspect.signature(net.forward).parameters
+        self._adacof_kwargs = {"return_sides": False} if "return_sides" in self._adacof_params else {}
 
     def _state(self, h, w):
         key = (h, w)
@@ -59,28 +60,37 @@
         h, w = rgb_frame1.shape[1:]
         pyr, phase_net = self._state(h, w)
         nlev = pyr.height - 2
-        lab12 = torch.empty((6, h, w), dtype=torch.float32, device=rgb_frame1.device)
+        fin = None
+        if ops.lean_frame() and "frames_out" in self._adacof_params and h % 8 == 0 and w % 8 == 0:
+            fin = torch.empty((1, self.fusion_net.in_channels, h, w), dtype=torch.float32, device=rgb_frame1.device)
+        lab12 = fin[0, 9:15] if fin is not None else torch.empty((6, h, w), dtype=torch.float32, device=rgb_frame1.device)
         ops.rgb2lab(rgb_frame1, out=lab12[:3])
         ops.rgb2lab(rgb_frame2, out=lab12[3:])
         f1, f2 = rgb_frame1.unsqueeze(0), rgb_frame2.unsqueeze(0)
-        return self._run(rgb_frame1, rgb_frame2, output_baseline, pyr, phase_net, nlev, lab12, f1, f2)
+        return self._run(rgb_frame1, rgb_frame2, output_baseline, pyr, phase_net, nlev, lab12, f1, f2, fin)
 
-    def _run(self, rgb_frame1, rgb_frame2, output_baseline, pyr, phase_net, nlev, lab12, f1, f2):
+    def _run(self, rgb_frame1, rgb_frame2, output_baseline, pyr, phase_net, nlev, lab12, f1, f2, fin=None):
         h, w = rgb_frame1.shape[1:]
         vals, bufs, amp_max = pyr.filter(lab12, concat_frames=2, phase_scale=1.0 / math.pi,
                                          amp_max_eps=phase_net.eps)
         vals_pred = phase_net(phase_net.normalize_vals(vals, concat=bufs, amp_max=amp_max))
         lab_pred = pyr.inv_filter(DecompValues(0, vals_pred.phase, vals_pred.amplitude, vals_pred.low_level))
-        phase_pred = ops.lab2rgb(lab_pred)
+        phase_pred = ops.lab2rgb(lab_pred, out=fin[0, 6:9] if fin is not None else None)
         pp = phase_pred.unsqueeze(0)
+        maps = fin[:, 15:18] if fin is not None else torch.empty((1, 3, h, w), dtype=torch.float32, device=rgb_frame1.device)
 
-        _, _, three, masks = self.adacof(torch.cat((f1, f1, pp), 0), torch.cat((f2, pp, f2), 0), **self._adacof_kwargs)
-        ada_pred, flow_var_map, between = three[:1], masks[:1], three[1:]
+        if fin is not None:
+            ada_pred, flow_var_map = fin[:, 3:6], maps[:, 2:3]
+            between = torch.empty((2, 3, h, w), dtype=torch.float32, device=rgb_frame1.device)
+            self.adacof([f1, f1, pp], [f2, pp, f2], return_sides=False, frames_out=[ada_pred, between[:1], between[1:]],
+                        masks_out=[flow_var_map, None, None])
+        else:
+            _, _, three, masks = self.adacof(torch.cat((f1, f1, pp), 0), torch.cat((f2, pp, f2), 0), **self._adacof_kwargs)
+            ada_pred, flow_var_map, between = three[:1], masks[:1], three[1:]
 
         coarse = min(6, nlev)
         m = ops.channel_mean_diff(ada_pred, phase_pred.unsqueeze(0), 1.0, False, signed=True)
         hf = pyr.band_filter(m, level_mask=1, keep_high=True)
-        maps = torch.empty((1, 3, h, w), dtype=torch.float32, device=rgb_frame1.device)
         d = ops.absdiff(hf, None, 100.0, True)
         phase_uncertainty = ops.gaussian_filter(d, 5, out=maps[:, 1])
         mask = ((1 << coarse) - 1) << (nlev - coarse)
@@ -95,7 +105,11 @@
         fd = ops.channel_mean_diff(freq.unsqueeze(0), None, 30.0, False)
         ada_uncertainty = ops.absdiff(fd, ops.median_filter(fd, 50), 5.0, True, out=maps[:, 0])
 
-        _, _, base, _ = self.adacof(between[:1], between[1:], **self._adacof_kwargs)
+        if fin is not None:
+            base = fin[:, 0:3]
+            self.adacof([between[:1]], [between[1:]], return_sides=False, frames_out=[base])
+        else:
+            _, _, base, _ = self.adacof(between[:1], between[1:], **self._adacof_kwargs)
 
         out = {"phase_pred": pp, "ada_pred": ada_pred, "base": base, "flow_var_map": flow_var_map,
                "phase_uncertainty": phase_uncertainty, "ada_uncertainty": ada_uncertainty}
@@ -107,8 +121,11 @@
             out["baseline"] = ops.lab2rgb(lab).unsqueeze(0)
 
         other = lab12.unsqueeze(0)
-        maps[:, 2].copy_(flow_var_map[:, 0])
-        out["final"] = self.fusion_net(base, ada_pred, pp, other, maps, variant=0)
+        if fin is None:
+            maps[:, 2].copy_(flow_var_map[:, 0])
+            out["final"] = self.fusion_net(base, ada_pred, pp, other, maps, variant=0)
+        else:
+            out["final"] = self.fusion_net(base, ada_pred, pp, other, maps, variant=0, assembled=fin)
         return out
 
 
diff --git a/fusion-method-for-video-frame-interpolation_amd/vfi_amd/ops.py b/fusion-method-for-video-frame-interpolation_amd/vfi_amd/ops.py
--- a/fusion-method-for-video-frame-interpolation_amd/vfi_amd/ops.py
+++ b/fusion-method-for-video-frame-interpolation_amd/vfi_amd/ops.py
@@ -1,3 +1,4 @@
+import ctypes
 import os
 
 import torch
@@ -58,7 +59,12 @@
 
 
 WINOGRAD = os.environ.get("VFI_CONV_WINOGRAD", "1") != "0"
+STREAM1X1 = os.environ.get("VFI_CONV_STREAM1X1", "1") != "0"
 FUSED_RESIZE = (not WINOGRAD) or os.environ.get("VFI_CONV_FUSED_RESIZE", "0") == "1"
+def lean_frame():
+    return os.environ.get("VFI_FRAME_LEAN", "1") != "0"
+
+
 def _winograd_work(n, cin, cout, h, w, residual=False, pooled=False, act="relu"):
     algo = _lib.lib().vfi_conv2d_algo(n, cin, h, w, cout, 3, int(bool(residual)), int(bool(pooled)), ACT[act])
     if algo == 2:
@@ -119,11 +125,12 @@
     return out
 
 
-def conv2d_pool2(x, pc, is_max, pad_mode="zeros", act="relu"):
+def conv2d_pool2(x, pc, is_max, pad_mode="zeros", act="relu", pooled_only=False):
     n, cin, h, w = x.shape
     if cin != pc.cin:
         raise VfiLibraryError(f"conv2d_pool2: input has {cin} channels, weights expect {pc.cin}")
-    out, pooled = new((n, pc.cout, h, w), x), new((n, pc.cout, h // 2, w // 2), x)
+    lean = pooled_only and pc.ks == 3 and WINOGRAD and act == "relu" and (cin + 3) // 4 < 16
+    out, pooled = None if lean else new((n, pc.cout, h, w), x), new((n, pc.cout, h // 2, w // 2), x)
     xp, xs = _slice_ptr(x, "x")
     ws = _workspace(x.device)
     work = None
@@ -133,8 +140,8 @@
         else:
             work = ("flop", 2.0 * n * cin * pc.cout * pc.ks * pc.ks * h * w,
                     f"conv2d_mfma_kernel<{pc.ks},{4 if pc.ks == 5 else 8},{2 if ((pc.cout + 31) // 32 * 32) % 64 == 0 else 1}>")
-    _lib.call("vfi_conv2d_pool2", xp, xs, pc.packed.data_ptr(), pc.bias.data_ptr(), out.data_ptr(), out.stride(0),
-              pooled.data_ptr(), pooled.stride(0), int(bool(is_max)), n, cin, h, w, pc.cout, pc.ks, PAD[pad_mode], ACT[act],
+    _lib.call("vfi_conv2d_pool2", xp, xs, pc.packed.data_ptr(), pc.bias.data_ptr(), None if lean else out.data_ptr(),
+              0 if lean else out.stride(0), pooled.data_ptr(), pooled.stride(0), int(bool(is_max)), n, cin, h, w, pc.cout, pc.ks, PAD[pad_mode], ACT[act],
               ws.data_ptr(), ws.numel(), _lib.stream_ptr(), work=work)
     return out, pooled
 
@@ -161,7 +168,30 @@
     return out
 
 
+def sample_ptrs(tensors):
+    if len(tensors) > 8:
+        raise VfiLibraryError(f"per-sample pointers: {len(tensors)} samples (at most 8)")
+    return (ctypes.c_void_p * len(tensors))(*[None if t is None else t.data_ptr() for t in tensors])
+
+
 def adacof_prepare(frame0, frame2, rgbx=True):
+    if isinstance(frame0, (list, tuple)):
+        n = len(frame0)
+        shape3 = tuple(frame0[0].shape[-3:])
+        for t in (*frame0, *frame2):
+            if not t.is_cuda or t.dtype != torch.float32 or tuple(t.shape[-3:]) != shape3 or t.numel() != 3 * shape3[1] * shape3[2] or not t.is_contiguous():
+                raise VfiLibraryError("adacof_prepare: per-sample frames must be dense float32 (3,H,W) tensors of one size on a HIP device")
+        if shape3[0] != 3 or len(frame2) != n:
+            raise VfiLibraryError("adacof_prepare: frames must both be N x (3,H,W)")
+        h, w = shape3[1:]
+        hp, wp = (h + 31) // 32 * 32, (w + 31) // 32 * 32
+        shape = (n, hp, wp, 4) if rgbx else (n, 3, hp, wp)
+        like = frame0[0]
+        pad0, pad2, x6 = new(shape, like), new(shape, like), new((n, 6, hp, wp), like)
+        p0, p2 = sample_ptrs(frame0), sample_ptrs(frame2)
+        _lib.call("vfi_adacof_prepare_ptrs", ctypes.addressof(p0), ctypes.addressof(p2), pad0.data_ptr(), pad2.data_ptr(), x6.data_ptr(),
+                  n, h, w, hp, wp, int(bool(rgbx)), _lib.stream_ptr())
+        return pad0, pad2, x6
     n, c, h, w = frame0.shape
     if c != 3 or tuple(frame2.shape) != tuple(frame0.shape):
         raise VfiLibraryError("adacof_prepare: frames must both be (N,3,H,W)")
@@ -1149,10 +1179,10 @@
     return out
 
 
-def lab2rgb(lab):
+def lab2rgb(lab, out=None):
     x = lab.contiguous()
     hw = x.shape[-1] * x.shape[-2]
-    out = torch.empty_like(x)
+    out = _out_like(x, out, "lab2rgb")
     _lib.call("vfi_lab2rgb", _lib.dptr(x, "lab"), out.data_ptr(), x.numel() // (3 * hw), hw, _lib.stream_ptr())
     return out
 
diff --git a/fusion-method-for-video-frame-interpolation_amd/vfi_amd/phase_net/phase_net.py b/fusion-method-for-video-frame-interpolation_amd/vfi_amd/phase_net/phase_net.py
--- a/fusion-method-for-video-frame-interpolation_amd/vfi_amd/phase_net/phase_net.py
+++ b/fusion-method-for-video-frame-interpolation_amd/vfi_amd/phase_net/phase_net.py
@@ -203,7 +203,8 @@
             if not fused and not filled:
                 ops.resize_bilinear(fp, (h, w), align_corners=False, out=x[:, :64 + p_prev])
             tail = tail_on and idx + 1 < m and h * w >= tail_min and packed[layer(idx + 1)][0].ks == 3 and (64 + p_band) % 8 == 0
-            fp = block(i, x, ops.new((b, 64 if tail else 64 + p_band, h, w), low_in), prev=fp if fused and not filled else None, head=False)
+            top = n_img == 2 and idx + 1 == m and h * w >= 4096 and h * w % 2 == 0 and ops.STREAM1X1 and ops.lean_frame()
+            fp = block(i, x, ops.new((b, 64 if tail or top else 64 + p_band, h, w), low_in), prev=fp if fused and not filled else None, head=False)
             amp_in = x[:, 64 + p_prev + c:]
             cp = packed[i][2]
             if cp.cout != p_band or cp.ks != 1:
@@ -215,9 +216,9 @@
             elif n_img == 2:
                 p_out, a_out = ops.new((b * 4, 1, h, w), low_in), ops.new((b * 4, 1, h, w), low_in)
                 _lib.call("vfi_phasenet_predict", fp.data_ptr(), fp.stride(0), cp.packed.data_ptr(), cp.bias.data_ptr(), amp_in.data_ptr(),
-                          x.stride(0), self.max_amplitudes[idx].data_ptr(), fp[:, 64:].data_ptr(), fp.stride(0), p_out.data_ptr(),
-                          a_out.data_ptr(), b, 64, h, w, stream,
-                          work=("byte", 4.0 * b * (64 + 8 + 8 + 8) * h * w, "phasenet_predict_kernel") if _lib.PROFILE is not None else None)
+                          x.stride(0), self.max_amplitudes[idx].data_ptr(), None if top else fp[:, 64:].data_ptr(), fp.stride(0),
+                          p_out.data_ptr(), a_out.data_ptr(), b, 64, h, w, stream,
+                          work=("byte", 4.0 * b * (64 + 8 + 8 + (0 if top else 8)) * h * w, "phasenet_predict_kernel") if _lib.PROFILE is not None else None)
             else:
                 if c != 4 * n_img:
                     raise RuntimeError(f"PhaseNet(num_img={n_img}): level {idx} has {c} phase planes, expected {4 * n_img}")
diff --git a/include/vfi_hip.h b/include/vfi_hip.h
--- a/include/vfi_hip.h
+++ b/include/vfi_hip.h
@@ -51,6 +51,13 @@
                           float *out_t1, float *out_t2, float *out_frame, float *out_mask,
                           int N, int H, int W, int F, int dilation, int weights_are_logits, vfi_stream_t stream);
 
+#define VFI_MAX_SAMPLE_PTRS 8
+
+int vfi_adacof_fused_rgbx_crop(const float *frame0_rgbx, const float *frame2_rgbx, const float *w1, const float *a1,
+                               const float *b1, const float *w2, const float *a2, const float *b2, const float *occ,
+                               float *const *out_frames, long long frame_cstride, float *const *out_masks, int N, int H,
+                               int W, int h0, int w0, int F, int dilation, vfi_stream_t stream);
+
 
 typedef enum vfi_act {
     VFI_ACT_NONE = 0,
@@ -95,6 +102,9 @@
 int vfi_adacof_prepare(const float *frame0, const float *frame2, float *pad0, float *pad2, float *x6, int N,
                        int H, int W, int Hp, int Wp, int rgbx, vfi_stream_t stream);
 
+int vfi_adacof_prepare_ptrs(const float *const *frames0, const float *const *frames2, float *pad0, float *pad2, float *x6,
+                            int N, int H, int W, int Hp, int Wp, int rgbx, vfi_stream_t stream);
+
 int vfi_pool2(const float *x, long long x_bstride, float *y, long long y_bstride, int N, int C, int H, int W,
               int is_max, vfi_stream_t stream);
 
```

New measurement: 26.18 frames/s (median of 6 runs). No clear change (+0.9%).
